# LRMPUT/PUTSLAM

Measured on AMD Instinct MI355X. Metric: frame-pairs/s (match+RANSAC+Kabsch), 640x480 @ 2000 kpts, higher is better.
Workload: dtype f32; 1 GPU; BASELINE configs[2]: TUM fr1/desk-style synthetic sequence, 500 frames = 499 frame pairs per step per GPU, 2000 kpts/frame, 256-bit descriptors, Hamming BF + cross-check -> depth filter -> H=4096 3-pt Umeyama hypotheses (fixed) scored with errorVersion 1 -> refit; inputs resident in HBM; kpts=2000, hypotheses=4096, world_size=1, force_dist=False, estimator=fixed, streams=4, join=end, submit=ps_batch_queue_submit: whole batches to the library's chains in turn, matcher_kernel=mfma-fused, score_kernel=fast, hw_queues=4, accepted_pairs=499

## Files before the change

putslam_amd/csrc/ps_capi.hip:

```cpp
#include "ps_kernels.h"
#include "ps_matcher_mfma.h"
#include "ps_score_fast.h"
#include "ps_score_euclid.h"
#include "ps_internal.h"
#include "ps_glue.h"

#include <cfloat>
#include <chrono>
#include <climits>
#include <cmath>
#include <cstdio>
#include <cstdlib>
#include <cstring>
#include <string>
#include <vector>

using namespace psdev;

static_assert(kPsReorderMargin == kReorderMargin && kPsReorderTopMax == kReorderTopMax, "ps_internal.h mirrors ps_score_fast.h");

namespace {

constexpr int kWidePairs = 16;
constexpr int kListRsplit3 = 4, kReorderGran = 64, kReorderC2div = 16;
// ... 81 lines not shown

int effective_mode(int errorVersion)
{
    switch (errorVersion) {
    case PS_EUCLIDEAN_ERROR:
    case PS_REPROJECTION_ERROR:
    case PS_EUCLIDEAN_AND_REPROJECTION_ERROR:
    case PS_ADAPTIVE_ERROR:
        return errorVersion;
    default:
        return PS_MAHALANOBIS_ERROR;
    }
}

enum class Scoring { Value, Euclid, Reproj };

struct Plan {
    int mode = 0;
    Scoring score = Scoring::Value;
    int H = 0;
    int minRun = 3;
    ScoreConsts sc{};
    FastConsts fc{};
    EuclidConsts ec{};
    PrepArgs pa{};
    SelectArgs sa{};
    ModelArgs ma{};
    int msplit = 1;
    bool genSplit = false;
    bool genPlain = false;
    bool reorder = false;
    bool prune = false;
    bool bailWatch = false;
    int bailSlot = 0;
    int prefix = 0;
    int lastStage = 0;
    bool big0 = false;
};

int make_plan(PsContext *ctx, const PsRansacParams *prm, const PsRansacConfig *cfg, const float *K, int cap,
              int trainRange, Plan &pl)
{
    if (!prm || !cfg) return fail(ctx, PS_ERR_BAD_ARG, "null params/config");
    if (prm->usedPairs != 3) return fail(ctx, PS_ERR_UNSUPPORTED, "usedPairs must be 3");
    if (cfg->numHypotheses < 1 || cfg->numHypotheses > PS_MAX_HYPOTHESES)
        return fail(ctx, PS_ERR_BAD_ARG, "numHypotheses out of range");
    if (cfg->estimator < PS_EST_RANSAC || cfg->estimator > PS_EST_FIXED)
        return fail(ctx, PS_ERR_BAD_ARG, "unknown estimator");
    pl.mode = effective_mode(prm->errorVersion);
    if (ctx->scoreFast == 0 || pl.mode == PS_MAHALANOBIS_ERROR) pl.score = Scoring::Value;
    else pl.score = (pl.mode == PS_EUCLIDEAN_ERROR || pl.mode == PS_ADAPTIVE_ERROR) ? Scoring::Euclid : Scoring::Reproj;
    float k[9] = {0, 0, 0, 0, 0, 0, 0, 0, 0};
    if (K) memcpy(k, K, sizeof k);
    pl.sc.fx = k[0]; pl.sc.fy = k[4]; pl.sc.cx = k[2]; pl.sc.cy = k[5];
    pl.sc.boundR = sq_bound_f64(prm->inlierThresholdReprojection);
    pl.sc.bLo = -1.0f;
    pl.sc.bHi = INFINITY;
    if (pl.sc.boundR >= 1e-20 && pl.sc.boundR <= 1e30) {
        const double w = 4.76837158203125e-07;
        double lo = pl.sc.boundR * (1.0 - w), hi = pl.sc.boundR * (1.0 + w);
        float flo = (float)lo, fhi = (float)hi;
        if ((double)flo > lo) flo = std::nextafterf(flo, 0.0f);
        if ((double)fhi < hi) fhi = std::nextafterf(fhi, INFINITY);
        pl.sc.bLo = flo;
        pl.sc.bHi = fhi;
    }
    {
        FastConsts &fc = pl.fc;
        const double fm = std::fmax(std::fmax(std::fabs((double)k[0]), std::fabs((double)k[4])), 1.0);
        const double cm = std::fmax(std::fabs((double)k[2]), std::fabs((double)k[5]));
        const double bR = pl.sc.boundR;
        fc.enabled = (bR >= 1e-12 && bR <= 1e12 && fm <= 1e6 && cm <= 1e6) ? 1 : 0;
        if (fc.enabled) {
            const double T = std::sqrt(bR);
            auto up = [](double v) { float f = (float)v; return (double)f < v ? std::nextafterf(f, INFINITY) : f; };
            auto down = [](double v) { float f = (float)v; return (double)f > v ? std::nextafterf(f, -INFINITY) : f; };
            fc.fmaxK = up(fm);
            fc.cmaxK = up(cm);
            fc.thrUp = up(T * (1.0 + 1e-5));
            fc.bIn0 = down(bR * (1.0 - 20.0 * 5.9604644775390625e-08));
            fc.cIn = up(2.0 * std::sqrt(2.0) * T * (1.0 + 1e-5));
            const double c = std::sqrt(2.0) * (1.0 + 1e-5);
            fc.thr2Up = up((double)fc.thrUp * (double)fc.thrUp);
            fc.cHi = up((2.0 * c + c * c) * (double)fc.thrUp);
        }
    }
    {
        EuclidConsts &ec = pl.ec;
        const double thr = prm->inlierThresholdEuclidean;
        ec.enabled = (thr >= 1e-10 && thr <= 1e10) ? 1 : 0;
        ec.tbLo = ec.tbHi = 0.0f;
        if (ec.enabled) {
            const double u = 5.9604644775390625e-08;
            auto up = [](double v) { float f = (float)v; return (double)f < v ? std::nextafterf(f, INFINITY) : f; };
            auto down = [](double v) { float f = (float)v; return (double)f > v ? std::nextafterf(f, -INFINITY) : f; };
            if (pl.mode == PS_ADAPTIVE_ERROR) {
                ec.tbLo = down(thr * (1.0 - 7.0 * u));
                ec.tbHi = up(thr * (1.0 + 7.0 * u));
            } else {
                const double Tb = std::sqrt((double)sq_bound_f32(thr));
                ec.tbLo = down(Tb * (1.0 - 6.0 * u));
                ec.tbHi = up(Tb * (1.0 + 6.0 * u));
            }
        }
    }
    pl.pa.fx = k[0]; pl.pa.fy = k[4]; pl.pa.cx = k[2]; pl.pa.cy = k[5];
    pl.pa.thrE = prm->inlierThresholdEuclidean;
    pl.pa.mode = pl.mode;
    pl.pa.cap = cap;
    pl.sa.estimator = cfg->estimator;
    pl.sa.mode = pl.mode;
    pl.sa.cap = cap;
    pl.sa.minMatches = (cfg->estimator == PS_EST_USAC) ? 8 : prm->minimalNumberOfMatches;
    pl.sa.minRatio = prm->minimalInlierRatioThreshold;
    pl.sa.trainRange = trainRange;
    pl.minRun = pl.sa.minMatches > 3 ? pl.sa.minMatches : 3;
    int H = cfg->numHypotheses;
    if (cfg->estimator == PS_EST_RANSAC) {
        int a = ransac_iterations_host(0.20), b = ransac_iterations_host(prm->minimalInlierRatioThreshold);
        int most = a > b ? a : b;
        if (most < H) H = most;
        if (H < 1) H = 1;
    } else if (cfg->estimator == PS_EST_USAC) {
        if (H > (int)kUsacMaxHyp) H = (int)kUsacMaxHyp;
    }
    pl.H = H;
    pl.sa.H = H;
    int rc = prepare_tables(ctx, cfg->estimator, prm->minimalInlierRatioThreshold, H, pl.sa);
    if (rc != PS_OK) return rc;
    if (pl.sa.iter0 > H) pl.sa.iter0 = H;
    pl.ma.seed = cfg->seed;
    pl.ma.raw = nullptr;
    pl.ma.seedDev = nullptr;
    return PS_OK;
}

void tick(PsContext *ctx, int slot, bool stop)
{
    if (!ctx->timing || slot >= kMaxTimed || ctx->ev.empty()) return;
    (void)hipEventRecord(ctx->ev[((size_t)ctx->curCall * kMaxTimed + slot) * 2 + (stop ? 1 : 0)], ctx->stream);
    if (stop) {
        ctx->slotMask[ctx->curCall] |= 1u << slot;
        if (slot + 1 > ctx->nTimed) ctx->nTimed = slot + 1;
    }
}

RecPtrs rec_ptrs(PsContext *ctx, Scoring score)
{
    RecPtrs r;
    r.G = score == Scoring::Euclid ? (float *)ctx->recF.p : nullptr;
    r.A = (float4 *)ctx->recA.p; r.B = (float4 *)ctx->recB.p; r.C = (float4 *)ctx->recC.p; r.D = (int4 *)ctx->recD.p;
    r.E = (float4 *)ctx->recE.p;
    r.F = (float2 *)ctx->recF.p;
#ifdef PS_STREAM_DIAG
    r.S = (float4 *)ctx->recShadow.p;
#endif
    return r;
}

int pick_split(long long blocksWithout, int maxSplit, int minChunkOf, int total)
{
    const long long want = 2048;
    if (blocksWithout >= want) return 1;
    long long s = (want + blocksWithout - 1) / (blocksWithout > 0 ? blocksWithout : 1);
    if (s > maxSplit) s = maxSplit;
    while (s > 1 && total / s < minChunkOf) --s;
    return (int)(s < 1 ? 1 : s);
}

template <int MODE>
void launch_score(PsContext *ctx, dim3 grid, const Plan &pl, int cap, int msplit)
{
    hipLaunchKernelGGL(ps_ransac_score<MODE>, grid, dim3(kBlock), 0, ctx->stream, (const float4 *)ctx->recA.p,
                       (const float4 *)ctx->recB.p, (const float4 *)ctx->recC.p, (const int32_t *)ctx->mvalid.p,
                       (const float2 *)ctx->cmax.p, pl.ma, pl.sc, pl.H, cap, pl.minRun, msplit, (int32_t *)ctx->counts.p);
}

unsigned big_limit(int mode) { return mode == PS_REPROJECTION_ERROR ? 1536u : 1280u; }

int prepare_score(PsContext *ctx, Plan &pl, int P, int cap, bool complete = false, bool adaptive = false, const void *dataKey = nullptr)
{
    const int H = pl.H;
    const int hb = (H + kBlock - 1) / kBlock;
    const bool prunable = pl.score != Scoring::Value;
    const size_t mbytes = (size_t)P * H * 12 * sizeof(float);
    pl.prefix = pl.sa.estimator == PS_EST_FIXED ? kPrefixFixed : kPrefixAdaptive;
    if (ctx->forcePrefix > 0 && pl.sa.estimator == PS_EST_FIXED) pl.prefix = ctx->forcePrefix;
    const double units = (double)P * (double)(hb - 1) * (double)cap;
    const StagedFrom sf = pl.score == Scoring::Euclid ? (pl.sa.estimator == PS_EST_FIXED ? kStagedFromEuclidFixed : kStagedFromEuclidAdaptive)
                                                      : (pl.sa.estimator == PS_EST_FIXED ? kStagedFromReprojFixed : kStagedFromReprojAdaptive);
    double stagedFrom = sf.base + sf.perRow * (double)cap;
    if (ctx->sideBySide >= 2) {
        const StagedFrom sb = pl.score == Scoring::Euclid ? (pl.sa.estimator == PS_EST_FIXED ? kStagedFromEuclidFixedSbs : kStagedFromEuclidAdaptiveSbs)
                                                          : (pl.sa.estimator == PS_EST_FIXED ? kStagedFromReprojFixedSbs : kStagedFromReprojAdaptiveSbs);
        const double sbs = sb.base + sb.perRow * (double)cap;
        stagedFrom = ctx->sideBySide >= 3 ? sbs : std::sqrt(sbs * stagedFrom);
    }
    pl.prune = !complete && ctx->prune != 0 && prunable && H > kPrefixFixed && (ctx->prune == 2 || units >= stagedFrom);
    pl.bailWatch = false;
    pl.bailSlot = 0;
    const bool willReorder = ctx->reorder == 1 || (ctx->reorder == 2 && pl.sa.estimator == PS_EST_FIXED);
    if (adaptive && pl.prune && willReorder && ctx->bail != 0 && pl.score == Scoring::Euclid && pl.sa.estimator == PS_EST_FIXED) {
        if (!ctx->bailHost) {
            const size_t nb = (size_t)PsContext::kBailKinds * 2 * sizeof(unsigned);
            if (hipHostMalloc((void **)&ctx->bailHost, nb, hipHostMallocMapped) == hipSuccess &&
                hipHostGetDevicePointer((void **)&ctx->bailHostDev, ctx->bailHost, 0) == hipSuccess) {
                memset(ctx->bailHost, 0, nb);
                if (ensure(ctx, ctx->bailCnt, nb) == PS_OK) (void)hipMemsetAsync(ctx->bailCnt.p, 0, nb, ctx->stream);
            } else {
                (void)hipGetLastError();
                ctx->bailHostDev = nullptr;
            }
        }
        if (ctx->bailHostDev && ctx->bailCnt.p) {
            int pclass = 0;
            for (int q = P; q > 1; q >>= 1) ++pclass;
            int slot = -1, lru = 0;
            for (int i = 0; i < PsContext::kBailKinds; ++i) {
                const PsContext::BailKind &b = ctx->bailKinds[i];
                if (b.mode == pl.mode && b.estimator == pl.sa.estimator && b.H == H && b.pclass == pclass && b.cap == cap && b.frames == dataKey) slot = i;
                if (b.used < ctx->bailKinds[lru].used) lru = i;
            }
            if (slot < 0) {
                slot = lru;
                PsContext::BailKind &b = ctx->bailKinds[slot];
                b.mode = pl.mode; b.estimator = pl.sa.estimator; b.H = H; b.pclass = pclass; b.cap = cap; b.frames = dataKey;
                b.hopeless = 0;
                b.calls = 0;
                (void)hipStreamSynchronize(ctx->stream);
                b.seen[0] = ((volatile unsigned *)ctx->bailHost)[2 * slot];
                b.seen[1] = ((volatile unsigned *)ctx->bailHost)[2 * slot + 1];
            }
            PsContext::BailKind &b = ctx->bailKinds[slot];
            b.used = ++ctx->bailClock;
            const unsigned s0 = ((volatile unsigned *)ctx->bailHost)[2 * slot], s1 = ((volatile unsigned *)ctx->bailHost)[2 * slot + 1];
            if (s0 != b.seen[0]) {
                const unsigned d0 = s0 - b.seen[0], d1 = s1 - b.seen[1];
                const int was = b.hopeless;
                b.hopeless = (2ull * d1 > d0) ? 1 : 0;
                if (b.hopeless != was) b.calls = 0;
                b.seen[0] = s0;
                b.seen[1] = s1;
            }
            if (b.hopeless && (++b.calls & 15) != 0)
                pl.prune = false;
            pl.bailWatch = pl.prune;
            pl.bailSlot = slot;
            ctx->bailSlot = slot;
            ctx->hopeless = b.hopeless;
        }
    }
    if (adaptive && !pl.prune && (double)P * (double)H * (double)cap > 2.0e14)
        return fail(ctx, PS_ERR_UNSUPPORTED, "complete scoring of this batch (pairs x hypotheses x matches > 2e14) would run for minutes: "
                                             "leave the staged scoring on (option \"prune\") or pass fewer pairs per call");
    PS_ENSURE(ctx->counts, (size_t)P * H * sizeof(int32_t));
    pl.msplit = pick_split((long long)P * (pl.prune ? 1 : hb), 32, 64, cap);
    pl.genSplit = pl.prune && ctx->genSplit != 0 && pl.msplit > 1;
    if (pl.genSplit) pl.msplit = pl.msplit * 2 < 32 ? pl.msplit * 2 : 32;
    if (ctx->forceMsplit > 0) pl.msplit = ctx->forceMsplit;
    if (pl.msplit <= 1) pl.genSplit = false;
    pl.pa.zeroCounts = pl.msplit > 1 ? (int32_t *)ctx->counts.p : nullptr;
    pl.pa.zeroH = pl.prune ? pl.prefix : H;
    pl.pa.zeroStride = H;
    pl.ma.models = nullptr;
    pl.ma.modelH = H;
    pl.lastStage = (pl.sa.estimator != PS_EST_FIXED && !willReorder && ctx->singleRest != 0) ? 1 : kStages;
    if (pl.prune) {
        const size_t room = ctx->modelRoomMiB > 0 ? ((size_t)ctx->modelRoomMiB << 20)
                                                  : (pl.sa.estimator == PS_EST_FIXED ? ((size_t)2 << 30) : ((size_t)256 << 20));
        if (mbytes > room) {
            long long fit = (long long)(room / ((size_t)P * 12 * sizeof(float))) & ~(long long)(kBlock - 1);
            pl.ma.modelH = (int)(fit < kPrefixFixed ? kPrefixFixed : fit);
        }
    }
    if ((P <= kWidePairs && mbytes <= ((size_t)64 << 20)) || pl.prune) {
        PS_ENSURE(ctx->models, (size_t)P * pl.ma.modelH * 12 * sizeof(float));
        pl.ma.models = (float *)ctx->models.p;
    }
    pl.genPlain = false;
    if (!pl.prune && pl.score != Scoring::Value && ctx->genSplit != 0 && pl.msplit > 1 && P >= kGenPlainFrom && mbytes <= ((size_t)1 << 30)) {
        PS_ENSURE(ctx->models, mbytes);
        pl.ma.models = (float *)ctx->models.p;
        PS_ENSURE(ctx->validMask, (size_t)P * ((H + 63) / 64) * sizeof(unsigned long long));
        pl.genPlain = true;
    }
    pl.pa.zeroSurvA = pl.pa.zeroSurvB = nullptr;
    pl.big0 = (unsigned)pl.msplit * (unsigned)P * (pl.prune ? 1u : (unsigned)hb) > big_limit(pl.mode);
    pl.pa.skipF = !(pl.score == Scoring::Reproj && (pl.prune || pl.big0));
    pl.pa.skipE = !(pl.score == Scoring::Reproj && !pl.big0);
    if (pl.prune) {
        if (pl.lastStage > 1) {
            PS_ENSURE(ctx->survA, (size_t)P * pl.ma.modelH * sizeof(int32_t));
            PS_ENSURE(ctx->survB, (size_t)P * pl.ma.modelH * sizeof(int32_t));
        }
        PS_ENSURE(ctx->survN, (size_t)2 * P * sizeof(int32_t));
        if (pl.genSplit) PS_ENSURE(ctx->validMask, (size_t)P * ((pl.prefix + 63) / 64) * sizeof(unsigned long long));
        pl.reorder = ctx->reorder == 1 || (ctx->reorder == 2 && pl.sa.estimator == PS_EST_FIXED);
        if (pl.reorder) {
            const size_t n = (size_t)P * cap;
            PS_ENSURE(ctx->recF2, n * 40 > (size_t)P * ((cap + 1) / 2) * 64 ? n * 40 : (size_t)P * ((cap + 1) / 2) * 64);
            PS_ENSURE(ctx->permBuf, n * sizeof(int32_t));
            PS_ENSURE(ctx->prefInfo, (size_t)4 * P * sizeof(int32_t));
            PS_ENSURE(ctx->frontRec, (size_t)P * ((cap + 1) / 2) * 10 * sizeof(float));
        }
        pl.pa.zeroSurvA = (int32_t *)ctx->survN.p;
        pl.pa.zeroSurvB = (int32_t *)ctx->survN.p + P;
    }
    ctx->lastModelH = pl.ma.models ? pl.ma.modelH : 0;
    ctx->stagedP = pl.prune ? P : 0;
    ctx->stagedCap = pl.prune ? cap : 0;
    ctx->reorderedP = (pl.prune && pl.reorder) ? P : 0;
    return PS_OK;
}

struct K3Call {
    PsContext *ctx;
    const Plan &pl;
    int P, cap;
    const float2 *hotF;
    unsigned long long *dbg;
};

template <int KIND, bool LOOP = false> struct Kind {};

template <int MODE> struct EuclidK3 {
    const K3Call &c;
    template <int KIND, bool LOOP> void operator()(Kind<KIND, LOOP>, const StageArgs &st, unsigned groups, int msplit) const
    {
        PsContext *ctx = c.ctx;
        hipLaunchKernelGGL((ps_ransac_score_euclid<MODE, KIND, LOOP>), dim3(groups * (unsigned)msplit * (unsigned)c.P), dim3(kBlock),
                           0, ctx->stream, (const float4 *)ctx->recA.p, (const float4 *)ctx->recB.p,
                           KIND >= 1 ? c.hotF : (const float2 *)ctx->recF.p, (const int32_t *)ctx->mvalid.p,
                           (const float2 *)ctx->cmax.p, c.pl.ma, c.pl.sc, c.pl.ec, c.pl.sa, st, c.pl.H, c.cap, c.pl.minRun, msplit,
                           (int32_t *)ctx->counts.p, c.dbg);
    }
};

template <int MODE> struct ReprojK3 {
    const K3Call &c;
    template <bool BIG, int KIND, bool LOOP> void launch(const StageArgs &st, unsigned groups, int msplit) const
    {
        PsContext *ctx = c.ctx;
        hipLaunchKernelGGL((ps_ransac_score_fast<MODE, BIG, KIND, LOOP>), dim3(groups * (unsigned)msplit * (unsigned)c.P),
                           dim3(kBlock), 0, ctx->stream, (const float4 *)ctx->recA.p, (const float4 *)ctx->recB.p,
                           (const float4 *)ctx->recC.p, st.frontRec ? (const float4 *)st.frontRec : (const float4 *)ctx->recE.p,
                           KIND >= 1 ? c.hotF : (const float2 *)ctx->recF.p, (const int32_t *)ctx->mvalid.p,
                           (const float2 *)ctx->cmax.p, c.pl.ma, c.pl.sc, c.pl.fc, c.pl.ec, c.pl.sa, st, c.pl.H, c.cap, c.pl.minRun,
                           msplit, (int32_t *)ctx->counts.p, c.dbg);
    }
    template <int KIND, bool LOOP> void operator()(Kind<KIND, LOOP>, const StageArgs &st, unsigned groups, int msplit) const
    {
        if constexpr (KIND == 0) {
            if (!c.pl.big0) return launch<false, KIND, LOOP>(st, groups, msplit);
        }
        launch<true, KIND, LOOP>(st, groups, msplit);
    }
};

template <int MODE, class K3> void score_schedule(const K3Call &c, const K3 &k3)
{
    PsContext *ctx = c.ctx;
    const Plan &pl = c.pl;
    const int P = c.P;
    auto groups = [](int hCount) { return (unsigned)((hCount + kBlock - 1) / kBlock); };
    if (!pl.prune) {
        StageArgs st{};
        st.hCount = pl.H;
        if (pl.genPlain) {
            st.validMask = (unsigned long long *)ctx->validMask.p;
            st.genOnly = 1;
            k3(Kind<0>{}, st, groups(pl.H), 1);
            st.genOnly = 0;
        }
        k3(Kind<0>{}, st, groups(pl.H), pl.msplit);
        return;
    }
    auto list_groups = [&](int stage) {
        const int listed = (pl.H < pl.ma.modelH ? pl.H : pl.ma.modelH) - pl.prefix;
        const int all = ((listed > 0 ? listed : 1) + kBlock - 1) / kBlock;
        const int auto3 = all / 8 > 1 ? all / 8 : 1;
        const int auto2 = pl.score == Scoring::Euclid ? (all / 8 > 2 ? all / 8 : 2) : 64;
        const int want = pl.reorder ? (stage == 2 ? (ctx->listGroups2 > 0 ? ctx->listGroups2 : auto2)
                                                  : auto3) : all;
        return want < all ? want : all;
    };
    auto list_rsplit = [&](int stage) { return (pl.reorder && stage == kStages) ? kListRsplit3 : 1; };
    const bool usePretest = pl.reorder && ctx->pretest != 0 &&
                            (pl.mode == PS_EUCLIDEAN_AND_REPROJECTION_ERROR || pl.mode == PS_REPROJECTION_ERROR);
    const int blocks1 = (pl.H - pl.prefix + kBlock - 1) / kBlock;
    int loopGroups = 0;
    if (pl.sa.estimator != PS_EST_FIXED && blocks1 > 64) {
        loopGroups = (4096 + P - 1) / P;
        loopGroups = loopGroups < 4 ? 4 : loopGroups;
        loopGroups = loopGroups > blocks1 ? blocks1 : loopGroups;
    }
    auto stage_args = [&](int stage) {
        StageArgs st{};
        st.stage = stage;
        st.hBase = stage == 0 ? 0 : pl.prefix;
        st.hCount = stage == 0 ? pl.prefix : pl.H - pl.prefix;
        if (stage >= 2) st.hCount = list_groups(stage) * kBlock;
        int32_t *nA = (int32_t *)ctx->survN.p, *nB = nA + P;
        if (stage == 1) { st.listOut = (int32_t *)ctx->survA.p; st.countOut = nA; }
        if (stage == 2) { st.listIn = (const int32_t *)ctx->survA.p; st.countIn = nA; st.listOut = (int32_t *)ctx->survB.p; st.countOut = nB; }
        if (stage == 3) { st.listIn = (const int32_t *)ctx->survB.p; st.countIn = nB; }
        if (stage >= 1 && pl.reorder) st.perm = (const int32_t *)ctx->permBuf.p;
        if (stage >= 1 && pl.reorder) st.prefInfo = (const int32_t *)ctx->prefInfo.p;
        if (stage == 1 && usePretest) st.frontRec = (const float2 *)ctx->frontRec.p;
        st.listStride = pl.ma.modelH;
        st.loopGroups = stage == 1 ? loopGroups : 0;
        st.single = pl.lastStage == 1 ? 1 : 0;
        st.margin = ctx->reorderMargin;
        st.gran = kReorderGran;
        st.c2div = kReorderC2div;
        return st;
    };
    auto stage0_args = [&](bool gen) {
        StageArgs st = stage_args(0);
        if (pl.genSplit) {
            st.validMask = (unsigned long long *)ctx->validMask.p;
            st.genOnly = gen ? 1 : 0;
        }
        return st;
    };
    if (pl.genSplit) k3(Kind<0>{}, stage0_args(true), groups(pl.prefix), 1);
    k3(Kind<0>{}, stage0_args(false), groups(pl.prefix), pl.msplit);
    if (pl.reorder)
        hipLaunchKernelGGL(ps_stage_reorder<MODE>, dim3((unsigned)P), dim3(kBlock), 0, ctx->stream, (const float4 *)ctx->recA.p,
                           (const float4 *)ctx->recB.p, (const float4 *)ctx->recC.p, (const float2 *)ctx->recF.p,
                           (const int32_t *)ctx->mvalid.p, pl.ma, pl.sc, pl.sa, pl.prefix, ctx->reorderTop,
                           (ctx->bail != 0 && pl.score == Scoring::Euclid) ? 64 : 0, ctx->reorderMargin, pl.H, c.cap, pl.minRun,
                           (const int32_t *)ctx->counts.p, (float2 *)ctx->recF2.p, (int32_t *)ctx->permBuf.p,
                           (int32_t *)ctx->prefInfo.p, usePretest ? (float2 *)ctx->frontRec.p : (float2 *)nullptr,
                           pl.bailWatch ? (unsigned *)ctx->bailCnt.p + 2 * pl.bailSlot : (unsigned *)nullptr);
    if (loopGroups > 0)
        k3(Kind<1, true>{}, stage_args(1), (unsigned)loopGroups, 1);
    else
        k3(Kind<1>{}, stage_args(1), groups(pl.H - pl.prefix), 1);
    for (int sg = 2; sg <= pl.lastStage; ++sg) k3(Kind<2>{}, stage_args(sg), (unsigned)list_groups(sg), list_rsplit(sg));
}

template <int MODE> void launch_k3(const K3Call &c)
{
    if constexpr (MODE == PS_EUCLIDEAN_ERROR || MODE == PS_ADAPTIVE_ERROR) {
        if (c.pl.score == Scoring::Euclid) return score_schedule<MODE>(c, EuclidK3<MODE>{c});
    }
    if constexpr (MODE == PS_REPROJECTION_ERROR || MODE == PS_EUCLIDEAN_AND_REPROJECTION_ERROR) {
        if (c.pl.score == Scoring::Reproj) return score_schedule<MODE>(c, ReprojK3<MODE>{c});
    }
    launch_score<MODE>(c.ctx, dim3((unsigned)((c.pl.H + kBlock - 1) / kBlock) * (unsigned)c.pl.msplit * (unsigned)c.P), c.pl, c.cap,
                       c.pl.msplit);
}

int run_ransac_stage(PsContext *ctx, const Plan &pl, int P, int cap, const PsDMatch *dMatches,
                     const int32_t *dNumMatches, int matchStride, float *dPose, uint8_t *dMask, PsRansacStats *dStats,
                     int slot0)
{
    PS_ENSURE(ctx->counts, (size_t)P * pl.H * sizeof(int32_t));
    PS_ENSURE(ctx->idxList, (size_t)P * cap * sizeof(int32_t));
    tick(ctx, slot0, false);
    unsigned long long *dbg = nullptr;
    if (ctx->scoreStats && pl.score != Scoring::Value) {
        PS_ENSURE(ctx->dbgCnt, 8 * sizeof(unsigned long long));
        PS_HIP(hipMemsetAsync(ctx->dbgCnt.p, 0, 8 * sizeof(unsigned long long), ctx->stream));
        dbg = (unsigned long long *)ctx->dbgCnt.p;
    }
    const K3Call c{ctx, pl, P, cap, (const float2 *)(pl.reorder ? ctx->recF2.p : ctx->recF.p), dbg};
    switch (pl.mode) {
    case PS_EUCLIDEAN_ERROR: launch_k3<PS_EUCLIDEAN_ERROR>(c); break;
    case PS_REPROJECTION_ERROR: launch_k3<PS_REPROJECTION_ERROR>(c); break;
    case PS_EUCLIDEAN_AND_REPROJECTION_ERROR: launch_k3<PS_EUCLIDEAN_AND_REPROJECTION_ERROR>(c); break;
    case PS_ADAPTIVE_ERROR: launch_k3<PS_ADAPTIVE_ERROR>(c); break;
    default: launch_k3<PS_MAHALANOBIS_ERROR>(c); break;
    }
    tick(ctx, slot0, true);
    PS_HIP(hipGetLastError());
    SelectArgs sa = pl.sa;
    const size_t bitmapBytes = (((2 * (size_t)((sa.trainRange + 31) / 32)) + 3) & ~(size_t)3) * sizeof(uint32_t);
    const size_t stageRoom = ((size_t)63 << 10) - bitmapBytes;
    sa.stageCap = cap < 1536 ? cap : 1536;
    if ((size_t)sa.stageCap * 32 > stageRoom) sa.stageCap = (int)(stageRoom / 32);
    size_t lds = bitmapBytes + (size_t)sa.stageCap * 8 * sizeof(float);
    tick(ctx, slot0 + 1, false);
    hipLaunchKernelGGL(ps_select_refit<kBlock>, dim3((unsigned)P), dim3(kBlock), lds, ctx->stream,
                       (const float4 *)ctx->recA.p, (const float4 *)ctx->recB.p, (const float4 *)ctx->recC.p,
                       (const int4 *)ctx->recD.p, (const int32_t *)ctx->mvalid.p, (const int32_t *)ctx->counts.p,
                       dMatches, dNumMatches, matchStride, pl.ma, pl.sc, sa, (int32_t *)ctx->idxList.p, dPose,
                       dMask, dStats, ctx->stampsOn ? (unsigned long long *)ctx->stamps.p : (unsigned long long *)nullptr,
                       (pl.bailWatch && pl.reorder) ? (const unsigned *)ctx->bailCnt.p + 2 * pl.bailSlot : (const unsigned *)nullptr,
                       (pl.bailWatch && pl.reorder) ? ctx->bailHostDev + 2 * pl.bailSlot : (unsigned *)nullptr);
    tick(ctx, slot0 + 1, true);
    PS_HIP(hipGetLastError());
    return PS_OK;
}

int ensure_records(PsContext *ctx, size_t P, size_t cap)
{
    const size_t n = P * cap;
    PS_ENSURE(ctx->recA, n * 16);
    PS_ENSURE(ctx->recB, n * 16);
    PS_ENSURE(ctx->recC, n * 16);
    PS_ENSURE(ctx->recD, n * 16);
    PS_ENSURE(ctx->recE, n * 16);
    PS_ENSURE(ctx->recF, n * 40 > P * ((cap + 1) / 2) * 64 ? n * 40 : P * ((cap + 1) / 2) * 64);
#ifdef PS_STREAM_DIAG
    static const bool shadow = std::getenv("PUTSLAM_HIP_DIAG_SHADOW_RECORDS") != nullptr && std::atoi(std::getenv("PUTSLAM_HIP_DIAG_SHADOW_RECORDS")) != 0;
    if (shadow) PS_ENSURE(ctx->recShadow, n * 7 * 16);
#endif
    return PS_OK;
}

template <bool REC, int BLK>
void launch_prep(PsContext *ctx, const PsFrameSet &fs, const int32_t *dPairs, int P, const PrepArgs &pa, const RecPtrs &rp,
                 PsDMatch *dMatches, int32_t *dNumMatches)
{
    hipLaunchKernelGGL((ps_crosscheck_prep<REC, BLK>), dim3((unsigned)P), dim3(BLK), (size_t)fs.maxKpts * sizeof(uint32_t), ctx->stream,
                       fs.pts, fs.nkpts, dPairs, (uint32_t *)ctx->keys.p, pa, dMatches, dNumMatches, rp, (int32_t *)ctx->mvalid.p,
                       (float2 *)ctx->cmax.p, ctx->stampsOn ? (unsigned long long *)ctx->stamps.p : (unsigned long long *)nullptr);
}

int run_match_stage(PsContext *ctx, const PsFrameSet &fs, const int32_t *dPairs, int P, const Plan *pl, PsDMatch *dMatches,
                    int32_t *dNumMatches, int slot0)
{
    const int cap = fs.maxKpts;
    FrameStrides strides;
    if (int rc = frame_strides(ctx, fs, true, fs.pts != nullptr, "frame set", strides)) return rc;
    const int fstrideDw = strides.descDwords();
    PrepArgs pa = pl ? pl->pa : PrepArgs{};
    if (!pl) pa.cap = cap;
    pa.ptsStride = strides.ptsFloats();
    PS_ENSURE(ctx->keys, (size_t)P * cap * sizeof(uint32_t));
    PS_ENSURE(ctx->mvalid, (size_t)P * sizeof(int32_t));
    PS_ENSURE(ctx->cmax, (size_t)P * sizeof(float2));
    if (pl) {
        int rc = ensure_records(ctx, (size_t)P, (size_t)cap);
        if (rc != PS_OK) return rc;
    }
    const bool useMfma = ctx->matcher == 1 || (ctx->matcher == 2 && (double)P * cap * cap > 2.0e7);
    ctx->matcherUsed = useMfma ? 1 : 0;
    const size_t keyBytes = (size_t)P * cap * sizeof(uint32_t);
    const size_t cleanBefore = ctx->keysCleanPtr == ctx->keys.p ? ctx->keysCleanBytes : 0;
    struct KeysInUse {
        PsContext *c;
        size_t restore;
        bool done = false;
        ~KeysInUse() { c->keysCleanBytes = done ? restore : 0; }
    } keysInUse{ctx, cleanBefore};
    if (useMfma) {
        constexpr int TT = kMfmaTT;
        const int tpf = (cap + kTileRows - 1) / kTileRows;
        const int groups = (tpf + kWavesPerWG * TT - 1) / (kWavesPerWG * TT);
        int qsplit = pick_split((long long)P * groups, tpf, 1, tpf);
        if (ctx->forceQsplit > 0) qsplit = ctx->forceQsplit < tpf ? ctx->forceQsplit : tpf;
        if (ctx->matcherFused) {
            if (ctx->forceQsplit <= 0 && (long long)P * groups >= 1024) qsplit = 1;
            if (qsplit > 1) {
                int rc = keys_clean(ctx, keyBytes);
                if (rc != PS_OK) return rc;
                keysInUse.restore = ctx->keysCleanBytes;
            }
            tick(ctx, 5, false);
            hipLaunchKernelGGL(ps_hamming_mfma_fused<TT>, dim3((unsigned)(groups * qsplit) * (unsigned)P), dim3(kBlock), 0,
                               ctx->stream, (const uint32_t *)fs.desc, fs.nkpts, dPairs, cap, fstrideDw, tpf, groups, qsplit,
                               (uint32_t *)ctx->keys.p);
            tick(ctx, 5, true);
            PS_HIP(hipGetLastError());
        } else {
        PS_ENSURE(ctx->xq, (size_t)P * tpf * kTileU4 * sizeof(uint4));
        int xchunks = tpf < 8 ? tpf : 8;
        if ((long long)P * xchunks < 1024) xchunks = tpf < 64 ? tpf : 64;
        tick(ctx, 4, false);
        hipLaunchKernelGGL(ps_expand_query_fp4, dim3((unsigned)xchunks * (unsigned)P), dim3(kBlock), 0, ctx->stream,
                           (const uint32_t *)fs.desc, fs.nkpts, dPairs, cap, fstrideDw, tpf, xchunks, (uint4 *)ctx->xq.p,
                           qsplit > 1 ? (uint32_t *)ctx->keys.p : (uint32_t *)nullptr);
        tick(ctx, 4, true);
        tick(ctx, 5, false);
        hipLaunchKernelGGL(ps_hamming_mfma<TT>, dim3((unsigned)(groups * qsplit) * (unsigned)P), dim3(kBlock), 0,
                           ctx->stream, (const uint32_t *)fs.desc, fs.nkpts, dPairs, cap, fstrideDw, tpf, groups, qsplit,
                           (const uint4 *)ctx->xq.p, (uint32_t *)ctx->keys.p);
        tick(ctx, 5, true);
        PS_HIP(hipGetLastError());
        }
    } else {
        constexpr int TPL = 2;
        const int tiles = (cap + kBlock * TPL - 1) / (kBlock * TPL);
        int qsplit = pick_split((long long)P * tiles, 128, 16, cap);
        if (ctx->forceQsplit > 0) qsplit = ctx->forceQsplit;
        if (qsplit > 1) {
            int rc = keys_clean(ctx, keyBytes);
            if (rc != PS_OK) return rc;
            keysInUse.restore = ctx->keysCleanBytes;
        }
        tick(ctx, slot0, false);
        hipLaunchKernelGGL(ps_hamming_nn<TPL>, dim3((unsigned)(tiles * qsplit) * (unsigned)P), dim3(kBlock), 0, ctx->stream,
                           (const uint4 *)fs.desc, fs.nkpts, dPairs, cap, strides.descUint4(), tiles, qsplit, (uint32_t *)ctx->keys.p);
        tick(ctx, slot0, true);
        PS_HIP(hipGetLastError());
    }
    tick(ctx, slot0 + 1, false);
    const bool wide = P <= kWidePairs;
    const auto prep = pl ? (wide ? launch_prep<true, 1024> : launch_prep<true, kBlock>)
                         : (wide ? launch_prep<false, 1024> : launch_prep<false, kBlock>);
    prep(ctx, fs, dPairs, P, pa, pl ? rec_ptrs(ctx, pl->score) : RecPtrs{}, dMatches, dNumMatches);
    tick(ctx, slot0 + 1, true);
    PS_HIP(hipGetLastError());
    keysInUse.done = true;
    return PS_OK;
}

void identity16(float *T)
{
    for (int i = 0; i < 16; ++i) T[i] = (i % 5 == 0) ? 1.0f : 0.0f;
}

}

extern "C" {

int ps_match_hamming256(PsContext *ctx, const uint8_t *query, int nq, size_t qstep, const uint8_t *train, int nt,
                        size_t tstep, PsDMatch *out, int *nout)
{
    int rc = bind(ctx);
    if (rc) return rc;
    TimingOff toff(ctx);
    if (nout) *nout = 0;
    if (!out || !nout || nq < 0 || nt < 0 || (nq > 0 && !query) || (nt > 0 && !train))
        return fail(ctx, PS_ERR_BAD_ARG, "ps_match_hamming256: bad argument");
    if ((nq > 0 && qstep < PS_DESC_BYTES) || (nt > 0 && tstep < PS_DESC_BYTES))
        return fail(ctx, PS_ERR_UNSUPPORTED, "descriptor rows must be 32 bytes (ORB/LDB); float descriptors are out of scope");
    if (nq > PS_MAX_KPTS || nt > PS_MAX_KPTS) return fail(ctx, PS_ERR_UNSUPPORTED, "more than PS_MAX_KPTS rows");
    if (nq == 0 || nt == 0) return PS_OK;
    int cap = nq > nt ? nq : nt;
    PS_ENSURE(ctx->sDesc, (size_t)2 * cap * 32);
    PS_ENSURE(ctx->sNk, 2 * sizeof(int32_t) + 2 * sizeof(int32_t));
    PS_ENSURE(ctx->sMatches, (size_t)cap * sizeof(PsDMatch));
    PS_ENSURE(ctx->sNumM, sizeof(int32_t));
    uint8_t *dDesc = (uint8_t *)ctx->sDesc.p;
    PS_HIP(hipMemcpy2DAsync(dDesc, 32, query, qstep, 32, (size_t)nq, hipMemcpyHostToDevice, ctx->stream));
    PS_HIP(hipMemcpy2DAsync(dDesc + (size_t)cap * 32, 32, train, tstep, 32, (size_t)nt, hipMemcpyHostToDevice,
                            ctx->stream));
    int32_t hostMeta[4] = {nq, nt, 0, 1};
    PS_HIP(hipMemcpyAsync(ctx->sNk.p, hostMeta, sizeof hostMeta, hipMemcpyHostToDevice, ctx->stream));
    PsFrameSet fs;
    fs.desc = dDesc;
    fs.pts = nullptr;
    fs.nkpts = (const int32_t *)ctx->sNk.p;
    fs.numFrames = 2;
    fs.maxKpts = cap;
    fs.descFrameStride = fs.ptsFrameStride = 0;
    rc = run_match_stage(ctx, fs, (const int32_t *)ctx->sNk.p + 2, 1, nullptr, (PsDMatch *)ctx->sMatches.p, (int32_t *)ctx->sNumM.p, 0);
    if (rc) return rc;
    int32_t n = 0;
    PS_HIP(hipMemcpyAsync(&n, ctx->sNumM.p, sizeof n, hipMemcpyDeviceToHost, ctx->stream));
    PS_HIP(hipStreamSynchronize(ctx->stream));
    if (n > 0) {
        PS_HIP(hipMemcpyAsync(out, ctx->sMatches.p, (size_t)n * sizeof(PsDMatch), hipMemcpyDeviceToHost, ctx->stream));
        PS_HIP(hipStreamSynchronize(ctx->stream));
    }
    *nout = n;
    return PS_OK;
}

static int ransac_host_entry(PsContext *ctx, const PsRansacParams *params, const PsRansacConfig *cfg, const float *K,
                             const float *prev, int nprev, const float *cur, int ncur, const PsDMatch *matches, int m,
                             float *pose, PsDMatch *inliers, int *ninl, uint8_t *mask, PsRansacStats *stats,
                             int32_t *countsOut)
{
    int rc = bind(ctx);
    if (rc) return rc;
    TimingOff toff(ctx);
    PsRansacStats st;
    memset(&st, 0, sizeof st);
    st.bestHypothesis = -1;
    st.numMatchesIn = m > 0 ? m : 0;
    st.pointInlierRatio = NAN;
    if (pose) identity16(pose);
    if (ninl) *ninl = 0;
    if (stats) *stats = st;
    if (!pose || !ninl || m < 0 || nprev < 0 || ncur < 0 || (m > 0 && (!matches || !prev || !cur || !inliers)))
        return fail(ctx, PS_ERR_BAD_ARG, "ps_ransac_rigid3d: bad argument");
    if (mask && m > 0) memset(mask, 0, (size_t)m);
    if (m > (1 << 22)) return fail(ctx, PS_ERR_UNSUPPORTED, "too many matches");
    for (int i = 0; i < m; ++i)
        if (matches[i].queryIdx < 0 || matches[i].queryIdx >= nprev || matches[i].trainIdx < 0 ||
            matches[i].trainIdx >= ncur)
            return fail(ctx, PS_ERR_BAD_ARG, "match index out of range");
    const int cap = m > 0 ? m : 1;
    const int trainRange = ncur <= 65536 ? ncur : 0;
    Plan pl;
    rc = make_plan(ctx, params, cfg, K, cap, trainRange, pl);
    if (rc) return rc;
    if (cfg->sampleIdx) {
        PS_ENSURE(ctx->raw, (size_t)pl.H * 3 * sizeof(uint32_t));
        PS_HIP(hipMemcpyAsync(ctx->raw.p, cfg->sampleIdx, (size_t)pl.H * 3 * sizeof(uint32_t), hipMemcpyHostToDevice,
                              ctx->stream));
        pl.ma.raw = (const uint32_t *)ctx->raw.p;
    }
    rc = prepare_score(ctx, pl, 1, cap, countsOut != nullptr);
    if (rc) return rc;
    PS_ENSURE(ctx->sMisc0, (size_t)(nprev > 0 ? nprev : 1) * 12);
    PS_ENSURE(ctx->sMisc1, (size_t)(ncur > 0 ? ncur : 1) * 12);
    PS_ENSURE(ctx->sMatches, (size_t)cap * sizeof(PsDMatch));
    PS_ENSURE(ctx->sNumM, sizeof(int32_t));
    PS_ENSURE(ctx->sMask, (size_t)cap);
    PS_ENSURE(ctx->sPose, 16 * sizeof(float));
    PS_ENSURE(ctx->sStats, sizeof(PsRansacStats));
    PS_ENSURE(ctx->mvalid, sizeof(int32_t));
    PS_ENSURE(ctx->cmax, sizeof(float2));
    rc = ensure_records(ctx, 1, (size_t)cap);
    if (rc) return rc;
    if (nprev > 0) PS_HIP(hipMemcpyAsync(ctx->sMisc0.p, prev, (size_t)nprev * 12, hipMemcpyHostToDevice, ctx->stream));
    if (ncur > 0) PS_HIP(hipMemcpyAsync(ctx->sMisc1.p, cur, (size_t)ncur * 12, hipMemcpyHostToDevice, ctx->stream));
    if (m > 0)
        PS_HIP(hipMemcpyAsync(ctx->sMatches.p, matches, (size_t)m * sizeof(PsDMatch), hipMemcpyHostToDevice,
                              ctx->stream));
    int32_t mm = m;
    PS_HIP(hipMemcpyAsync(ctx->sNumM.p, &mm, sizeof mm, hipMemcpyHostToDevice, ctx->stream));
    hipLaunchKernelGGL(ps_prep_from_matches, dim3(1), dim3(kBlock), 0, ctx->stream, (const float *)ctx->sMisc0.p,
                       (const float *)ctx->sMisc1.p, (const PsDMatch *)ctx->sMatches.p, m, pl.pa, rec_ptrs(ctx, pl.score),
                       (int32_t *)ctx->mvalid.p, (float2 *)ctx->cmax.p);
    PS_HIP(hipGetLastError());
    rc = run_ransac_stage(ctx, pl, 1, cap, (const PsDMatch *)ctx->sMatches.p, (const int32_t *)ctx->sNumM.p, cap,
                          (float *)ctx->sPose.p, (uint8_t *)ctx->sMask.p, (PsRansacStats *)ctx->sStats.p, 2);
    if (rc) return rc;
    std::vector<uint8_t> hmask((size_t)cap);
    PS_HIP(hipMemcpyAsync(pose, ctx->sPose.p, 16 * sizeof(float), hipMemcpyDeviceToHost, ctx->stream));
    PS_HIP(hipMemcpyAsync(&st, ctx->sStats.p, sizeof st, hipMemcpyDeviceToHost, ctx->stream));
    if (m > 0) PS_HIP(hipMemcpyAsync(hmask.data(), ctx->sMask.p, (size_t)m, hipMemcpyDeviceToHost, ctx->stream));
    if (countsOut) {
        int32_t mv = 0;
        PS_HIP(hipMemcpyAsync(&mv, ctx->mvalid.p, sizeof mv, hipMemcpyDeviceToHost, ctx->stream));
        PS_HIP(hipStreamSynchronize(ctx->stream));
        if (mv >= pl.minRun)
            PS_HIP(hipMemcpyAsync(countsOut, ctx->counts.p, (size_t)pl.H * sizeof(int32_t), hipMemcpyDeviceToHost,
                                  ctx->stream));
        else
// ... 296 lines not shown
```

putslam_amd/csrc/ps_context.cpp:

```cpp
#include <cfloat>
#include <climits>
#include <cmath>
#include <cstdio>
#include <cstdlib>
#include <cstring>

#include "ps_internal.h"

int ransac_iterations_host(double inlierRatio, double successProbability, int numberOfPairs)
{
    double v = std::log(1 - successProbability) / std::log(1 - std::pow(inlierRatio, numberOfPairs));
    if (!(v < 2147483647.0)) return INT_MAX;
    if (v < 0) return 0;
    return (int)v;
}

unsigned usac_stopping_host(double prob_good_model)
{
    if (prob_good_model < DBL_EPSILON) return kUsacMaxHyp;
    if (1 - prob_good_model < DBL_EPSILON) return 1;
    double n = std::log(1 - 0.99) / std::log(1 - prob_good_model);
    return (unsigned)std::ceil(n);
}

void build_ransac_table(double minRatio, int H, std::vector<float> &tab, int &iter0, float &tiny)
{
    uint32_t tlo = 0, thi;
    {
        float probe = 1e-4f;
        memcpy(&thi, &probe, 4);
        while (thi - tlo > 1) {
            uint32_t mid = tlo + (thi - tlo) / 2;
            float mf;
            memcpy(&mf, &mid, 4);
            if (ransac_iterations_host((double)mf) == 0) tlo = mid; else thi = mid;
        }
        memcpy(&tiny, &tlo, 4);
    }
    int itersMin = ransac_iterations_host(minRatio);
    int kcap = itersMin < H ? itersMin : H;
    if (kcap < 0) kcap = 0;
    tab.resize((size_t)kcap);
    uint32_t one;
    float onef = 1.0f;
    memcpy(&one, &onef, 4);
    uint32_t hi = one;
    for (int k = 0; k < kcap; ++k) {
        uint32_t lo = thi;
        while (hi - lo > 1) {
            uint32_t mid = lo + (hi - lo) / 2;
            float mf;
            memcpy(&mf, &mid, 4);
            if (ransac_iterations_host((double)mf) <= k) hi = mid; else lo = mid;
        }
        memcpy(&tab[(size_t)k], &hi, 4);
    }
    int i0 = ransac_iterations_host(0.20);
    iter0 = i0 < H ? i0 : H;
}

void build_usac_table(int H, std::vector<double> &tab)
{
    int n = H < (int)kUsacMaxHyp ? H : (int)kUsacMaxHyp;
    tab.resize((size_t)(n > 0 ? n : 0));
    uint64_t oneb;
    double oned = 1.0;
    memcpy(&oneb, &oned, 8);
    uint64_t hiPrev = oneb;
    const double pFloor = 1.862645149230957e-09;
    uint64_t floorb;
    memcpy(&floorb, &pFloor, 8);
    for (int k = 0; k < n; ++k) {
        unsigned target = (unsigned)k + 1u;
        uint64_t lo = floorb, hi = hiPrev;
        if (target >= kUsacMaxHyp) {
            tab[(size_t)k] = 0.0;
            continue;
        }
        {
            const double ps = -std::expm1(std::log(1 - 0.99) / (double)target);
            const double a = ps * (1.0 - 1e-11), b = ps * (1.0 + 1e-11);
            uint64_t ab, bb;
            memcpy(&ab, &a, 8);
            memcpy(&bb, &b, 8);
            if (ab > lo && ab < hi && usac_stopping_host(a) > target) lo = ab;
            if (bb > lo && bb < hi && usac_stopping_host(b) <= target) hi = bb;
        }
        while (hi - lo > 1) {
            uint64_t mid = lo + (hi - lo) / 2;
            double md;
            memcpy(&md, &mid, 8);
            if (usac_stopping_host(md) <= target) hi = mid; else lo = mid;
        }
        memcpy(&tab[(size_t)k], &hi, 8);
        hiPrev = hi;
    }
}


namespace {

struct OptDesc {
    const char *name;
    const char *env;
    int PsContext::*field;
    int lo, hi;
    const char *what;
    bool shape = false;
};
const OptDesc kOptions[] = {
    {"matcher", "MATCHER", &PsContext::matcher, 0, 2, "matcher: 0 (VALU), 1 (MFMA) or 2 (by batch size)"},
    {"matcher_fused", "MATCHER_FUSED", &PsContext::matcherFused, 0, 1, "matcher_fused: 0 or 1"},
    {"matcher_l2", "MATCHER_L2", &PsContext::matcherL2, 0, 1, "matcher_l2: 0 (value-exact sweep) or 1 (matrix-core prefilter + value-exact evaluation)"},
    {"l2_stats", nullptr, &PsContext::l2Stats, 0, 1, "l2_stats: 0 or 1"},
    {"score", "SCORE", &PsContext::scoreFast, 0, 1, "score: 0 (value-exact kernels) or 1 (decision-exact kernels)"},
    {"score_stats", nullptr, &PsContext::scoreStats, 0, 1, "score_stats: 0 or 1"},
    {"prune", "PRUNE", &PsContext::prune, 0, 2, "prune: 0 (complete scoring), 1 (staged from the cost model's batch size on) or 2 (staged whenever possible)"},
    {"side_by_side", "SIDE_BY_SIDE", &PsContext::sideBySide, 0, 16, "side_by_side: 0 (the context runs alone) or the number of launch chains it shares the chip with"},
    {"reorder", "REORDER", &PsContext::reorder, 0, 2, "reorder: 0, 1 or 2"},
    {"qsplit", "QSPLIT", &PsContext::forceQsplit, 0, 1024, "qsplit: 0 (automatic) .. 1024", true},
    {"msplit", "MSPLIT", &PsContext::forceMsplit, 0, 1024, "msplit: 0 (automatic) .. 1024", true},
    {"gensplit", "GENSPLIT", &PsContext::genSplit, 0, 1, "gensplit: 0 (stage 0 as one launch) or 1 (models, then the sweep)", true},
    {"singlerest", "SINGLEREST", &PsContext::singleRest, 0, 1, "singlerest: 0 (three stages) or 1 (one stage after the prefix, adaptive schedules)", true},
    {"pretest", "PRETEST", &PsContext::pretest, 0, 1, "pretest: 0 or 1 (stage 1's one-direction pre-test)", true},
    {"list_g2", "LISTG2", &PsContext::listGroups2, 0, 64, "list_g2: 0 (automatic) .. 64 work-groups per pair of stage 2", true},
    {"prefix", "PREFIX", &PsContext::forcePrefix, 0, 256, "prefix: 0 (default) or 64, 128, 192, 256 hypotheses of stage 0 (fixed schedule)", true},
    {"reorder_top", "REORDER_TOP", &PsContext::reorderTop, 1, kPsReorderTopMax, "reorder_top: 1 .. 16 voters", true},
    {"reorder_margin", "REORDER_MARGIN", &PsContext::reorderMargin, 1, 4096, "reorder_margin: 1 .. 4096 matches", true},
    {"bail", "BAIL", &PsContext::bail, 0, 1, "bail: 0 or 1 (pairs whose prefix leaves nothing to abandon are swept in one stage)"},
    {"stream_copy_kernels", "STREAM_COPY_KERNELS", &PsContext::streamCopyKernels, 0, 1, "stream_copy_kernels: 0 (hipMemcpyAsync) or 1 (copy kernels over mapped pinned memory)"},
    {"stream_ahead", "STREAM_AHEAD", &PsContext::streamAhead, -1, 8, "stream_ahead: -1 (automatic: six places in all) or 0 .. 8 chunks the pipelined stream takes beyond one per lane (queued on the lanes' streams)"},
    {"model_room_mib", "MODEL_ROOM_MIB", &PsContext::modelRoomMiB, 0, 65536, "model_room_mib: 0 (default) .. 65536 MiB for the staged scoring's parked models"},
};
const OptDesc *find_option(const char *name)
{
    const bool dbg = strncmp(name, "debug.", 6) == 0;
    if (dbg) name += 6;
    for (const OptDesc &o : kOptions)
        if (o.shape == dbg && strcmp(name, o.name) == 0) return &o;
    return nullptr;
}
bool option_value_ok(const OptDesc &o, int v)
{
    if (v < o.lo || v > o.hi) return false;
    if (strcmp(o.name, "prefix") == 0) return (v & 63) == 0;
    return true;
}
int parse_option_text(const OptDesc &o, const char *v)
{
    if (strcmp(o.name, "score") == 0) {
        if (strcmp(v, "exact") == 0) return 0;
        if (strcmp(v, "fast") == 0) return 1;
    }
    if (strcmp(o.name, "matcher") == 0) {
        if (strcmp(v, "valu") == 0) return 0;
        if (strcmp(v, "mfma") == 0) return 1;
        if (strcmp(v, "auto") == 0) return 2;
    }
    char *end = nullptr;
    const long x = std::strtol(v, &end, 10);
    if (end == v || *end != '\0' || x < INT_MIN || x > INT_MAX) return INT_MIN;
    return (int)x;
}


}

int psi_options_snapshot(const PsContext *ctx, int *out, int cap)
{
    int n = 0;
    for (const OptDesc &o : kOptions)
        if (n < cap) out[n++] = ctx->*(o.field);
    return n;
}

extern "C" {

int ps_abi_version(void) { return PS_ABI_VERSION; }

size_t ps_abi_sizeof_dmatch(void) { return sizeof(PsDMatch); }
size_t ps_abi_sizeof_params(void) { return sizeof(PsRansacParams); }
size_t ps_abi_sizeof_config(void) { return sizeof(PsRansacConfig); }
size_t ps_abi_sizeof_stats(void) { return sizeof(PsRansacStats); }
size_t ps_abi_sizeof_frameset(void) { return sizeof(PsFrameSet); }
size_t ps_abi_sizeof_results(void) { return sizeof(PsPairResults); }
size_t ps_abi_sizeof_host_results(void) { return sizeof(PsHostPairResults); }

int ps_context_create(int device, PsContext **out)
{
    if (!out) return PS_ERR_BAD_ARG;
    *out = nullptr;
    int n = 0;
    hipError_t e = hipGetDeviceCount(&n);
    if (e != hipSuccess || n <= 0) return PS_ERR_NO_DEVICE;
    if (device < 0 || device >= n) return PS_ERR_BAD_ARG;
    if (hipSetDevice(device) != hipSuccess) return PS_ERR_HIP;
    PsContext *ctx = new PsContext();
    ctx->device = device;
    hipDeviceProp_t prop;
    if (hipGetDeviceProperties(&prop, device) == hipSuccess) {
        strncpy(ctx->arch, prop.gcnArchName, sizeof(ctx->arch) - 1);
    }
    if (hipStreamCreateWithFlags(&ctx->own, hipStreamNonBlocking) != hipSuccess) {
        delete ctx;
        return PS_ERR_HIP;
    }
    ctx->stream = ctx->own;
    for (const OptDesc &o : kOptions) {
        if (!o.env) continue;
        const std::string name = std::string("PUTSLAM_HIP_") + o.env;
        if (const char *v = std::getenv(name.c_str())) {
            const int x = parse_option_text(o, v);
            if (option_value_ok(o, x)) ctx->*(o.field) = x;
        }
    }
    psi_kernel_attributes();
    *out = ctx;
    return PS_OK;
}

void ps_context_destroy(PsContext *ctx)
{
    if (!ctx) return;
    (void)hipSetDevice(ctx->device);
    (void)hipStreamSynchronize(ctx->stream);
    Buf *all[] = {&ctx->keys, &ctx->recA, &ctx->recB, &ctx->recC, &ctx->recD, &ctx->recE, &ctx->recF, &ctx->recShadow, &ctx->models, &ctx->survA, &ctx->survB, &ctx->survN, &ctx->recF2, &ctx->permBuf, &ctx->prefInfo, &ctx->frontRec, &ctx->validMask, &ctx->stamps, &ctx->dbgCnt, &ctx->bailCnt, &ctx->counts, &ctx->mvalid,
                  &ctx->cmax, &ctx->idxList, &ctx->raw, &ctx->xq, &ctx->tabR, &ctx->tabU, &ctx->sDesc, &ctx->sNk,
                  &ctx->sMatches, &ctx->sNumM, &ctx->sMask, &ctx->sPose, &ctx->sStats,
                  &ctx->sMisc0, &ctx->sMisc1, &ctx->sMisc2, &ctx->exFlag, &ctx->exPar, &ctx->viewChunks, &ctx->levelTab, &ctx->poseSets, &ctx->loopPairs, &ctx->l2Keys, &ctx->l2Img, &ctx->l2Norms, &ctx->l2List, &ctx->l2ListLo, &ctx->l2Count, &ctx->l2Stat};
    for (Buf *b : all) release(*b);
    for (hipEvent_t e : ctx->ev)
        if (e) (void)hipEventDestroy(e);
    if (ctx->bailHost) (void)hipHostFree(ctx->bailHost);
    if (ctx->handoff) (void)hipEventDestroy(ctx->handoff);
    if (ctx->own) (void)hipStreamDestroy(ctx->own);
    delete ctx;
}

int ps_context_set_stream(PsContext *ctx, void *s)
{
    if (!ctx) return PS_ERR_BAD_ARG;
    hipStream_t next = s ? (hipStream_t)s : ctx->own;
    if (next == ctx->stream) return PS_OK;
    int rc = bind(ctx);
    if (rc) return rc;
    if (ctx->handoff && ctx->handoffPending) PS_HIP(hipStreamWaitEvent(next, ctx->handoff, 0));
    ctx->stream = next;
    return PS_OK;
}

void *ps_context_stream(PsContext *ctx) { return ctx ? (void *)ctx->stream : nullptr; }
int ps_context_device(const PsContext *ctx) { return ctx ? ctx->device : (int)PS_ERR_BAD_ARG; }

int ps_context_set_option(PsContext *ctx, const char *name, int value)
{
    if (!ctx || !name) return PS_ERR_BAD_ARG;
    if (strcmp(name, "stamps") == 0) {
        if (value != 0 && value != 1) return fail(ctx, PS_ERR_BAD_ARG, "stamps: 0 or 1");
        if (value) {
            int rc = bind(ctx);
            if (rc) return rc;
            PS_ENSURE(ctx->stamps, 16 * sizeof(unsigned long long));
            PS_HIP(hipMemsetAsync(ctx->stamps.p, 0, 16 * sizeof(unsigned long long), ctx->stream));
        }
        ctx->stampsOn = value;
        return PS_OK;
    }
    const OptDesc *o = find_option(name);
    if (!o) return fail(ctx, PS_ERR_BAD_ARG, "unknown option");
    if (!option_value_ok(*o, value)) return fail(ctx, PS_ERR_BAD_ARG, o->what);
    ctx->*(o->field) = value;
    if (strcmp(name, "bail") == 0) {
        for (PsContext::BailKind &b : ctx->bailKinds) b = PsContext::BailKind();
        ctx->hopeless = 0;
        ctx->bailSlot = -1;
    }
    return PS_OK;
}

int ps_context_get_option(const PsContext *ctx, const char *name)
{
    if (!ctx || !name) return PS_ERR_BAD_ARG;
    if (strcmp(name, "matcher_used") == 0) return ctx->matcherUsed;
    if (strcmp(name, "matcher_l2_used") == 0) return ctx->matcherL2Used;
    if (strcmp(name, "stamps") == 0) return ctx->stampsOn;
    if (strcmp(name, "last_staged_pairs") == 0) return ctx->stagedP;
    if (strcmp(name, "hopeless") == 0) return ctx->hopeless;
    if (strcmp(name, "arena_mib") == 0) {
        const Buf *all[] = {&ctx->keys, &ctx->recA, &ctx->recB, &ctx->recC, &ctx->recD, &ctx->recE, &ctx->recF, &ctx->models,
                            &ctx->survA, &ctx->survB, &ctx->survN, &ctx->recF2, &ctx->permBuf, &ctx->prefInfo, &ctx->frontRec,
                            &ctx->validMask, &ctx->stamps, &ctx->dbgCnt, &ctx->bailCnt, &ctx->counts, &ctx->mvalid, &ctx->cmax,
                            &ctx->idxList, &ctx->raw, &ctx->xq, &ctx->tabR, &ctx->tabU, &ctx->sDesc, &ctx->sNk, &ctx->sMatches,
                            &ctx->sNumM, &ctx->sMask, &ctx->sPose, &ctx->sStats, &ctx->sMisc0, &ctx->sMisc1, &ctx->sMisc2, &ctx->exFlag, &ctx->exPar, &ctx->viewChunks, &ctx->levelTab, &ctx->poseSets, &ctx->loopPairs, &ctx->l2Keys, &ctx->l2Img, &ctx->l2Norms, &ctx->l2List, &ctx->l2ListLo, &ctx->l2Count, &ctx->l2Stat};
        size_t sum = 0;
        for (const Buf *b : all) sum += b->cap;
        return (int)((sum + (((size_t)1 << 20) - 1)) >> 20);
    }
    if (strcmp(name, "hw_queues_seen") == 0) return psi_hw_queues_seen();
    if (strcmp(name, "last_model_slots") == 0) return ctx->lastModelH;
    if (strcmp(name, "last_reordered_pairs") == 0) return ctx->reorderedP;
    const OptDesc *o = find_option(name);
    return o ? ctx->*(o->field) : (int)PS_ERR_BAD_ARG;
}

int ps_context_synchronize(PsContext *ctx)
{
    int rc = bind(ctx);
    if (rc) return rc;
    PS_HIP(hipStreamSynchronize(ctx->stream));
    return PS_OK;
}

const char *ps_last_error(const PsContext *ctx) { return ctx ? ctx->err.c_str() : "null context"; }

void psi_set_error(PsContext *ctx, const char *what)
{
    if (ctx) ctx->err = what ? what : "";
}

void psi_copy_options(PsContext *dst, const PsContext *src)
{
    if (!dst || !src) return;
    for (const OptDesc &o : kOptions) dst->*(o.field) = src->*(o.field);
}
const char *ps_device_arch(const PsContext *ctx) { return ctx ? ctx->arch : ""; }

int ps_context_enable_timing(PsContext *ctx, int enable)
{
    int rc = bind(ctx);
    if (rc) return rc;
    if (enable && ctx->ev.empty()) {
        ctx->ev.assign((size_t)kTimingRing * kMaxTimed * 2, nullptr);
        for (hipEvent_t &e : ctx->ev) PS_HIP(hipEventCreate(&e));
    }
    ctx->timing = enable != 0;
    ctx->timedCalls = 0;
    ctx->curCall = 0;
    ctx->nTimed = 0;
    memset(ctx->slotMask, 0, sizeof ctx->slotMask);
    return PS_OK;
}

int ps_last_kernel_times_ms(PsContext *ctx, float *ms)
{
    int rc = bind(ctx);
    if (rc) return rc;
    if (!ctx->timing || ctx->timedCalls == 0) return 0;
    PS_HIP(hipStreamSynchronize(ctx->stream));
    for (int i = 0; i < ctx->nTimed; ++i) {
        float t = 0.f;
        size_t b = ((size_t)ctx->curCall * kMaxTimed + i) * 2;
        if (ctx->slotMask[ctx->curCall] & (1u << i)) PS_HIP(hipEventElapsedTime(&t, ctx->ev[b], ctx->ev[b + 1]));
        ms[i] = t;
    }
    return ctx->nTimed;
}

int ps_kernel_time_totals(PsContext *ctx, double *sum_ms, int *launches)
{
    int rc = bind(ctx);
    if (rc) return rc;
    for (int i = 0; i < kMaxTimed; ++i) {
        sum_ms[i] = 0.0;
        launches[i] = 0;
    }
    if (!ctx->timing || ctx->timedCalls == 0) return 0;
    PS_HIP(hipStreamSynchronize(ctx->stream));
    long long n = ctx->timedCalls < kTimingRing ? ctx->timedCalls : kTimingRing;
    for (long long c = 0; c < n; ++c)
        for (int i = 0; i < ctx->nTimed; ++i) {
            if (!(ctx->slotMask[c] & (1u << i))) continue;
            float t = 0.f;
            size_t b = ((size_t)c * kMaxTimed + i) * 2;
            PS_HIP(hipEventElapsedTime(&t, ctx->ev[b], ctx->ev[b + 1]));
            sum_ms[i] += t;
            launches[i] += 1;
        }
    return ctx->nTimed;
}

const char *ps_kernel_names(void)
{
    return "ps_hamming_nn\0ps_crosscheck_prep\0ps_ransac_score\0ps_select_refit\0ps_expand_query_fp4\0ps_hamming_mfma\0";
}

uint64_t ps_algorithmic_bytes(int nkpts, int matchesIn, int matchesValid, int H)
{
    return 2ull * nkpts * 32 + 16ull * matchesIn + 2ull * nkpts * 12 + 8ull * matchesValid + 12ull * H + 4ull * H +
           (uint64_t)matchesValid + 64ull;
}


int ps_predicted_level(int octave, double detDist, double curDist)
{
    const double scaleFactor = 1.2;
    const int nLevels = 8;
    const double logScaleFactor = std::log(scaleFactor);
    double detLevelScaleFactor = std::pow(scaleFactor, octave);
    double curLevelScaleFactor = detLevelScaleFactor * detDist / curDist;
    int curLevel = (int)std::ceil(std::log(curLevelScaleFactor) / logScaleFactor);
    if (curLevel < 0) curLevel = 0;
    if (curLevel > nLevels - 1) curLevel = nLevels - 1;
    return curLevel;
}

static bool level_above(double x, int k) { return std::ceil(std::log(x) / std::log(1.2)) > (double)k; }

int psi_level_tables(double *t7, double *pow64)
{
    static double T[7], P[PS_LEVEL_OCTAVE_MAX - PS_LEVEL_OCTAVE_MIN + 1];
    static int state = 0;
    if (state == 0) {
        auto bits = [](double d) { uint64_t b; std::memcpy(&b, &d, 8); return b; };
        auto val = [](uint64_t b) { double d; std::memcpy(&d, &b, 8); return d; };
        bool clean = true;
        for (int k = 0; k < 7 && clean; ++k) {
            uint64_t lo = bits(0.5), hi = bits(8.0);
            while (lo < hi) {
                const uint64_t mid = lo + (hi - lo) / 2;
                if (level_above(val(mid), k))
                    hi = mid;
                else
                    lo = mid + 1;
            }
            T[k] = val(lo);
            for (int64_t d = -4096; d <= 4096 && clean; ++d) clean = level_above(val(lo + (uint64_t)d), k) == (d >= 0);
        }
        for (int o = PS_LEVEL_OCTAVE_MIN; o <= PS_LEVEL_OCTAVE_MAX; ++o) P[o - PS_LEVEL_OCTAVE_MIN] = std::pow(1.2, o);
        state = clean ? 1 : -1;
    }
    if (state < 0) return PS_ERR_UNSUPPORTED;
    if (t7) std::memcpy(t7, T, sizeof(T));
    if (pow64) std::memcpy(pow64, P, sizeof(P));
    return PS_OK;
}

int ps_level_thresholds(double t[7])
{
    if (!t) return PS_ERR_BAD_ARG;
    return psi_level_tables(t, nullptr);
}

int ps_view_angles(const double *curPose16, const double *poses16, int numPoses, double *angle)
{
    if (!curPose16 || numPoses < 0 || (numPoses > 0 && (!poses16 || !angle))) return PS_ERR_BAD_ARG;
    const float a0 = (float)curPose16[8], a1 = (float)curPose16[9], a2 = (float)curPose16[10];
    const float na = std::sqrt(a0 * a0 + (a1 * a1 + a2 * a2));
    for (int q = 0; q < numPoses; ++q) {
        const double *m = poses16 + (size_t)q * 16;
        const float b0 = (float)m[8], b1 = (float)m[9], b2 = (float)m[10];
        const float dot = b0 * a0 + (b1 * a1 + b2 * a2);
        const float nb = std::sqrt(b0 * b0 + (b1 * b1 + b2 * b2));
        const float r = dot / (nb * na);
        angle[q] = std::fabs(std::acos((double)r));
    }
    return PS_OK;
}


}
```

putslam_amd/csrc/ps_internal.h:

```cpp
#pragma once
#include <hip/hip_runtime_api.h>

#include <cstddef>
#include <cstdint>
#include <string>
#include <vector>

#include "putslam_hip.h"

struct Buf {
    void *p = nullptr;
    size_t cap = 0;
};


constexpr int kMaxTimed = 8;
constexpr int kTimingRing = 128;

constexpr int kPsReorderMargin = 16, kPsReorderTopMax = 16;
constexpr unsigned kUsacMaxHyp = 850000u;

struct PsContext {
    int device = 0;
    hipStream_t own = nullptr;
    hipStream_t stream = nullptr;
    hipEvent_t handoff = nullptr;
    bool handoffPending = false;
    std::string err;
    char arch[64] = {0};
    Buf keys, recA, recB, recC, recD, recE, recF, counts, mvalid, cmax, idxList, raw;
    Buf models;
    Buf survA, survB, survN;
    Buf validMask;
    Buf frontRec;
    Buf prefInfo;
    Buf recF2, permBuf;
    Buf dbgCnt;
    Buf xq;
    Buf recShadow;
    Buf tabR, tabU;
    Buf sDesc, sNk, sMatches, sNumM, sMask, sPose, sStats, sMisc0, sMisc1, sMisc2;
    Buf exFlag, exPar;
    Buf viewChunks;
    Buf levelTab;
    Buf poseSets;
    Buf loopPairs;
    Buf l2Keys;
    Buf l2Img, l2Norms, l2List, l2ListLo, l2Count, l2Stat;
    int tabEstimator = -1, tabH = -1, tabRN = 0, tabUN = 0, tabIter0 = 0;
    double tabMinRatio = -1.0;
    float tabTiny = 0.0f;
    bool timing = false;
    std::vector<hipEvent_t> ev;
    long long timedCalls = 0;
    int curCall = 0;
    int nTimed = 0;
    unsigned slotMask[kTimingRing] = {0};
    int forceQsplit = 0, forceMsplit = 0;
    int matcher = 2;
    int matcherUsed = 1;
    int matcherFused = 1;
    int matcherL2 = 1;
    int matcherL2Used = 0;
    int l2Stats = 0;
    int scoreFast = 1;
    int scoreStats = 0;
    int prune = 1;
    int sideBySide = 0;
    int reorder = 2;
    int genSplit = 1;
    int singleRest = 1;
    int pretest = 1;
    int listGroups2 = 0;
    int forcePrefix = 0;
    int bail = 1;
    int streamCopyKernels = 1;
    int streamAhead = -1;
    int modelRoomMiB = 0;
    int reorderTop = 8, reorderMargin = kPsReorderMargin;
    int stampsOn = 0;
    Buf stamps;
    unsigned long long arenaGen = 0;
    int stagedP = 0, stagedCap = 0, reorderedP = 0;
    int lastModelH = 0;
    struct BailKind {
        int mode = -1, estimator = 0, H = 0, pclass = 0, cap = 0;
        const void *frames = nullptr;
        unsigned seen[2] = {0, 0};
        int hopeless = 0, calls = 0;
        unsigned long long used = 0;
    };
    static constexpr int kBailKinds = 8;
    BailKind bailKinds[kBailKinds];
    unsigned long long bailClock = 0;
    int bailSlot = -1;
    Buf bailCnt;
    unsigned *bailHost = nullptr;
    unsigned *bailHostDev = nullptr;
    int hopeless = 0;
    void *keysCleanPtr = nullptr;
    size_t keysCleanBytes = 0;
};


inline int fail(PsContext *c, int code, const char *what, hipError_t e = hipSuccess)
{
    if (c) {
        c->err = what;
        if (e != hipSuccess) {
            c->err += ": ";
            c->err += hipGetErrorString(e);
        }
    }
    return code;
}

#define PS_HIP(call)                                                  \
    do {                                                              \
        hipError_t e_ = (call);                                       \
        if (e_ != hipSuccess) return fail(ctx, PS_ERR_HIP, #call, e_); \
    } while (0)

inline int ensure(PsContext *ctx, Buf &b, size_t bytes)
{
    if (bytes <= b.cap) return PS_OK;
    size_t want = bytes + (bytes / 4 < ((size_t)16 << 20) ? bytes / 4 : ((size_t)16 << 20)) + 256;
    if (b.p) {
        hipError_t e = hipStreamSynchronize(ctx->stream);
        if (e != hipSuccess) return fail(ctx, PS_ERR_HIP, "hipStreamSynchronize", e);
        (void)hipFree(b.p);
        b.p = nullptr;
        b.cap = 0;
    }
    hipError_t e = hipMalloc(&b.p, want);
    if (e != hipSuccess) return fail(ctx, PS_ERR_ALLOC, "hipMalloc", e);
    b.cap = want;
    ctx->arenaGen++;
    return PS_OK;
}
#define PS_ENSURE(buf, bytes)                        \
    do {                                             \
        int rc_ = ensure(ctx, (buf), (bytes));       \
        if (rc_ != PS_OK) return rc_;                \
    } while (0)


inline void release(Buf &b)
{
    if (b.p) (void)hipFree(b.p);
    b.p = nullptr;
    b.cap = 0;
}


inline int bind(PsContext *ctx)
{
    if (!ctx) return PS_ERR_BAD_ARG;
    hipError_t e = hipSetDevice(ctx->device);
    if (e != hipSuccess) return fail(ctx, PS_ERR_HIP, "hipSetDevice", e);
    ctx->err.clear();
    return PS_OK;
}

int ransac_iterations_host(double inlierRatio, double successProbability = 0.98, int numberOfPairs = 3);
unsigned usac_stopping_host(double prob_good_model);
void build_ransac_table(double minRatio, int H, std::vector<float> &tab, int &iter0, float &tiny);
void build_usac_table(int H, std::vector<double> &tab);
int psi_options_snapshot(const PsContext *ctx, int *out, int cap);

extern "C" {
void psi_set_error(PsContext *ctx, const char *what);
void psi_copy_options(PsContext *dst, const PsContext *src);
int psi_hw_queues_seen(void);
int psi_hw_queues_defaulted(void);
void psi_kernel_attributes(void);
int psi_level_tables(double *t7, double *powTable);
}
```

putslam_amd/csrc/ps_kernels.h:

```cpp
#pragma once

#include "ps_device_math.h"

#include "../../include/putslam_hip.h"

namespace psdev {

constexpr int kBlock = 256;
constexpr uint32_t kNoKey = 0xFFFFFFFFu;

PS_D unsigned xcd_remap(unsigned L, unsigned total)
{
    const unsigned xcd = L & 7u, idx = L >> 3;
    const unsigned q = total >> 3, r = total & 7u;
    return (xcd < r ? xcd * (q + 1u) : r * (q + 1u) + (xcd - r) * q) + idx;
}

PS_D void phase_stamp(unsigned long long *stamps, int i)
{
    if (stamps != nullptr && threadIdx.x == 0 && blockIdx.x == 0) stamps[i] = __builtin_readcyclecounter();
}

PS_D uint32_t bcnt_acc(uint32_t x, uint32_t acc)
{
// ... 151 lines not shown
        const int sv = wsum[i];
        if (i < w) off += sv;
        tot += sv;
    }
    posA = (off & 0xFFFF) + __popcll(ba & below);
    posB = (off >> 16) + __popcll(bb & below);
    totalA = tot & 0xFFFF;
    totalB = tot >> 16;
}

template <int BLOCK = kBlock> PS_D void block_max2(float &a, float &b, float2 *red)
{
#pragma unroll
    for (int o = 32; o > 0; o >>= 1) {
        a = fmaxf(a, __shfl_down(a, o, 64));
        b = fmaxf(b, __shfl_down(b, o, 64));
    }
    if ((threadIdx.x & 63) == 0) red[threadIdx.x >> 6] = make_float2(a, b);
    __syncthreads();
    float2 r = red[0];
#pragma unroll
    for (int i = 1; i < BLOCK / 64; ++i) {
        r.x = fmaxf(r.x, red[i].x);
        r.y = fmaxf(r.y, red[i].y);
    }
    __syncthreads();
    a = r.x;
    b = r.y;
}

template <int BLOCK = kBlock> PS_D float block_max(float v, float *red)
{
#pragma unroll
    for (int o = 32; o > 0; o >>= 1) v = fmaxf(v, __shfl_down(v, o, 64));
    if ((threadIdx.x & 63) == 0) red[threadIdx.x >> 6] = v;
    __syncthreads();
    float r = red[0];
#pragma unroll
    for (int i = 1; i < BLOCK / 64; ++i) r = fmaxf(r, red[i]);
    __syncthreads();
    return r;
}

struct PrepArgs {
    float fx, fy, cx, cy;
    double thrE;
    int mode;
    int cap;
    int ptsStride;
    int32_t *zeroCounts;
    int zeroH;
    int zeroStride;
    int32_t *zeroSurvA, *zeroSurvB;
    int skipE, skipF;
};

struct RecPtrs {
    float4 *A;
    float4 *B;
    float4 *C;
    int4 *D;
    float4 *E;
#ifdef PS_STREAM_DIAG
    float4 *S;
#endif
    float2 *F;
    float *G;
};

PS_D float write_records(const PrepArgs &a, const RecPtrs &r, int p, int v, int srcIdx, int q, int t, float px, float py,
                         float pz, float cx_, float cy_, float cz_, float fixedBound)
{
    const float bound = a.mode == PS_ADAPTIVE_ERROR ? sq_bound_f32(a.thrE * (double)pz) : fixedBound;
    const size_t slot = (size_t)p * a.cap + (size_t)v;
    r.A[slot] = make_float4(px, py, pz, bound);
    r.B[slot] = make_float4(cx_, cy_, cz_, 1.0f);
    r.D[slot] = make_int4(srcIdx, q, t, 0);
    const bool euclidOnly = a.mode == PS_EUCLIDEAN_ERROR || a.mode == PS_ADAPTIVE_ERROR;
    float ou = 0.0f, ov = 0.0f, nu = 0.0f, nv = 0.0f;
    if (!euclidOnly) {
        project(px, py, pz, a.fx, a.fy, a.cx, a.cy, ou, ov);
        project(cx_, cy_, cz_, a.fx, a.fy, a.cx, a.cy, nu, nv);
        r.C[slot] = make_float4(ou, ov, nu, nv);
    }
    if (r.G != nullptr) {
        const bool adaptive = a.mode == PS_ADAPTIVE_ERROR;
        const int rf = adaptive ? 16 : 12;
        float *g = r.G + ((size_t)p * (size_t)((a.cap + 1) >> 1) + (size_t)(v >> 1)) * rf + (v & 1);
        if (adaptive) {
            const float w = 1.0f / pz;
            g[0] = cx_ * w; g[2] = cy_ * w; g[4] = cz_ * w; g[6] = w;
            g[8] = px * w; g[10] = py * w; g[12] = pz * w; g[14] = 0.0f;
        } else {
            g[0] = cx_; g[2] = cy_; g[4] = cz_;
            g[6] = px; g[8] = py; g[10] = pz;
        }
        return 0.0f;
    }
    if (euclidOnly) return 0.0f;
    const float4 e = make_float4(a.cx - ou, a.cx - nu, a.cy - ov, a.cy - nv);
    if (!a.skipE) r.E[slot] = e;
    if (!a.skipF) {
        float2 *f = r.F + 5 * slot;
        f[0] = make_float2(cx_, px); f[1] = make_float2(cy_, py); f[2] = make_float2(cz_, pz);
        f[3] = make_float2(e.x, e.y); f[4] = make_float2(e.z, e.w);
    }
#ifdef PS_STREAM_DIAG
    if (r.S != nullptr) {
        float4 *sh = r.S + 7 * slot;
        sh[0] = make_float4(px, py, pz, bound); sh[1] = make_float4(cx_, cy_, cz_, 1.0f); sh[2] = make_float4(ou, ov, nu, nv);
        sh[3] = make_float4((float)srcIdx, (float)q, (float)t, 0.0f); sh[4] = make_float4(cx_, px, cy_, py);
        sh[5] = make_float4(cz_, pz, e.x, e.y); sh[6] = make_float4(e.z, e.w, 0.0f, 0.0f);
    }
#endif
    const bool num = e.x == e.x && e.y == e.y && e.z == e.z && e.w == e.w;
    return num ? fmaxf(fmaxf(fabsf(e.x), fabsf(e.y)), fmaxf(fabsf(e.z), fabsf(e.w))) : INFINITY;
}

PS_D void finish_pair_records(const PrepArgs &a, const RecPtrs &r, int p, int M)
{
    if (r.G == nullptr || !(M & 1)) return;
    const int rf = a.mode == PS_ADAPTIVE_ERROR ? 16 : 12;
    float *g = r.G + ((size_t)p * (size_t)((a.cap + 1) >> 1) + (size_t)(M >> 1)) * rf;
    for (int i = 0; i < rf; i += 2) g[i + 1] = g[i];
}

template <bool WITH_RECORDS, int BLOCK = kBlock>
__global__ __launch_bounds__(BLOCK) void ps_crosscheck_prep(const float *__restrict__ pts,
                                                             const int32_t *__restrict__ nkpts,
                                                             const int32_t *__restrict__ pairs,
                                                             uint32_t *__restrict__ keys, PrepArgs a,
                                                             PsDMatch *__restrict__ matches,
                                                             int32_t *__restrict__ numMatches, RecPtrs rec,
                                                             int32_t *__restrict__ mvalid, float2 *__restrict__ cmaxOut,
                                                             unsigned long long *__restrict__ stamps)
{
    extern __shared__ __align__(16) uint32_t s_best[];
    phase_stamp(stamps, 0);
    __shared__ int s_wsum[2 * (BLOCK / 64)];
    __shared__ float2 s_red[BLOCK / 64];
    float cm = 0.0f;
    float um = 0.0f;
    const int p = blockIdx.x;
    const int cap = a.cap;
    const int fq = pairs[2 * p], ft = pairs[2 * p + 1];
    const int nq = nkpts[fq], nt = nkpts[ft];
    uint32_t k0 = kNoKey, k1 = kNoKey;
    if ((int)threadIdx.x < nt) k0 = keys[(size_t)p * cap + threadIdx.x];
    if ((int)threadIdx.x + BLOCK < nt) k1 = keys[(size_t)p * cap + threadIdx.x + BLOCK];
    for (int q = threadIdx.x; q < nq; q += BLOCK) s_best[q] = kNoKey;
    __syncthreads();
    for (int t = threadIdx.x; t < nt; t += BLOCK) {
        uint32_t key = t < BLOCK ? k0 : (t < 2 * BLOCK ? k1 : keys[(size_t)p * cap + t]);
        if (key != kNoKey) {
            uint32_t q = key & 0xFFFFu, d = key >> 16;
            atomicMin(&s_best[q], (d << 16) | (uint32_t)t);
            keys[(size_t)p * cap + t] = kNoKey;
        }
    }
    __syncthreads();
    phase_stamp(stamps, 1);
    const float *pp = pts + (size_t)fq * a.ptsStride;
    const float *cp = pts + (size_t)ft * a.ptsStride;
    int base = 0, vbase = 0;
    struct Cand {
        uint32_t key;
        float px, py, pz, cx, cy, cz;
    };
    auto fetch = [&](int q, Cand &c) {
        c.key = (q < nq) ? s_best[q] : kNoKey;
        c.px = c.py = c.pz = c.cx = c.cy = c.cz = 0.0f;
        if (WITH_RECORDS && c.key != kNoKey) {
            const int t = (int)(c.key & 0xFFFFu);
            c.px = pp[3 * q]; c.py = pp[3 * q + 1]; c.pz = pp[3 * q + 2];
            c.cx = cp[3 * t]; c.cy = cp[3 * t + 1]; c.cz = cp[3 * t + 2];
        }
    };
    const float fixedBound = (WITH_RECORDS && a.mode != PS_ADAPTIVE_ERROR) ? sq_bound_f32(a.thrE) : 0.0f;
    Cand cur;
    fetch((int)threadIdx.x, cur);
    int trip = 0;
    for (int q0 = 0; q0 < nq; q0 += BLOCK, ++trip) {
        const int q = q0 + threadIdx.x;
        Cand nxt;
        nxt.key = kNoKey;
        nxt.px = nxt.py = nxt.pz = nxt.cx = nxt.cy = nxt.cz = 0.0f;
        if (q0 + BLOCK < nq) fetch(q + BLOCK, nxt);
        const uint32_t key = cur.key;
        const bool has = key != kNoKey;
        const int t = (int)(key & 0xFFFFu);
        const float px = cur.px, py = cur.py, pz = cur.pz, cx_ = cur.cx, cy_ = cur.cy, cz_ = cur.cz;
        const bool ok = WITH_RECORDS && has && depth_ok(px, py, pz) && depth_ok(cx_, cy_, cz_);
        int pos, total, vpos, vtotal;
        block_scan_flags2_alt<BLOCK>(has, ok, pos, total, vpos, vtotal, s_wsum, trip);
        if (has) {
            PsDMatch m;
            m.queryIdx = q;
            m.trainIdx = t;
            m.imgIdx = 0;
            m.distance = (float)(key >> 16);
            matches[(size_t)p * cap + base + pos] = m;
        }
        if (WITH_RECORDS) {
            if (ok) {
                um = fmaxf(um, write_records(a, rec, p, vbase + vpos, base + pos, q, t, px, py, pz, cx_, cy_, cz_, fixedBound));
                cm = fmaxf(cm, fmaxf(fmaxf(fabsf(px), fabsf(py)), fmaxf(fabsf(pz), fmaxf(fabsf(cx_), fmaxf(fabsf(cy_), fabsf(cz_))))));
            }
            vbase += vtotal;
        }
        base += total;
        cur = nxt;
    }
    phase_stamp(stamps, 2);
    if (WITH_RECORDS) {
        float c = cm, u = um;
        block_max2<BLOCK>(c, u, s_red);
        if (threadIdx.x == 0) cmaxOut[p] = make_float2(c, u);
        if (threadIdx.x == 0) finish_pair_records(a, rec, p, vbase);
        if (a.zeroCounts)
            for (int i = threadIdx.x; i < a.zeroH; i += BLOCK) a.zeroCounts[(size_t)p * a.zeroStride + i] = 0;
    }
    if (threadIdx.x == 0) {
        numMatches[p] = base;
        if (WITH_RECORDS) mvalid[p] = vbase;
        if (WITH_RECORDS && a.zeroSurvA) {
            a.zeroSurvA[p] = 0;
            a.zeroSurvB[p] = 0;
        }
    }
    phase_stamp(stamps, 3);
}

__global__ __launch_bounds__(kBlock) void ps_prep_from_matches(const float *__restrict__ prev,
                                                               const float *__restrict__ cur,
                                                               const PsDMatch *__restrict__ matches, int m, PrepArgs a,
                                                               RecPtrs rec, int32_t *__restrict__ mvalid,
                                                               float2 *__restrict__ cmaxOut)
{
    __shared__ int s_wsum[kBlock / 64];
    __shared__ float s_red[kBlock / 64];
    float cm = 0.0f, um = 0.0f;
    int vbase = 0;
    const float fixedBound = a.mode != PS_ADAPTIVE_ERROR ? sq_bound_f32(a.thrE) : 0.0f;
    for (int i0 = 0; i0 < m; i0 += kBlock) {
        const int i = i0 + threadIdx.x;
        float px = 0, py = 0, pz = 0, cx_ = 0, cy_ = 0, cz_ = 0;
        int q = 0, t = 0;
        bool ok = false;
        if (i < m) {
            q = matches[i].queryIdx;
            t = matches[i].trainIdx;
            px = prev[3 * q]; py = prev[3 * q + 1]; pz = prev[3 * q + 2];
            cx_ = cur[3 * t]; cy_ = cur[3 * t + 1]; cz_ = cur[3 * t + 2];
            ok = depth_ok(px, py, pz) && depth_ok(cx_, cy_, cz_);
        }
        int vtotal;
        int vpos = block_scan_flag(ok, vtotal, s_wsum);
        if (ok) {
            um = fmaxf(um, write_records(a, rec, 0, vbase + vpos, i, q, t, px, py, pz, cx_, cy_, cz_, fixedBound));
            cm = fmaxf(cm, fmaxf(fmaxf(fabsf(px), fabsf(py)), fmaxf(fabsf(pz), fmaxf(fabsf(cx_), fmaxf(fabsf(cy_), fabsf(cz_))))));
        }
        vbase += vtotal;
    }
    float c = block_max(cm, s_red);
    float u = block_max(um, s_red);
    if (threadIdx.x == 0) {
        mvalid[0] = vbase;
        cmaxOut[0] = make_float2(c, u);
        finish_pair_records(a, rec, 0, vbase);
    }
    if (a.zeroCounts)
        for (int i = threadIdx.x; i < a.zeroH; i += kBlock) a.zeroCounts[i] = 0;
    if (threadIdx.x == 0 && a.zeroSurvA) {
        a.zeroSurvA[0] = 0;
        a.zeroSurvB[0] = 0;
    }
}

struct ModelArgs {
    uint64_t seed;
    const uint32_t *raw;
    const uint64_t *seedDev;
    float *models;
    int modelH;
};

PS_D void store_model(const ModelArgs &ma, size_t slot, const Rigid &m)
{
    float4 *d = reinterpret_cast<float4 *>(ma.models + slot * 12);
    d[0] = make_float4(m.R[0][0], m.R[0][1], m.R[0][2], m.R[1][0]);
    d[1] = make_float4(m.R[1][1], m.R[1][2], m.R[2][0], m.R[2][1]);
    d[2] = make_float4(m.R[2][2], m.t[0], m.t[1], m.t[2]);
}
PS_D void load_model(const ModelArgs &ma, size_t slot, Rigid &m)
{
    const float4 *d = reinterpret_cast<const float4 *>(ma.models + slot * 12);
    const float4 a = d[0], b = d[1], c = d[2];
    m.R[0][0] = a.x; m.R[0][1] = a.y; m.R[0][2] = a.z; m.R[1][0] = a.w;
    m.R[1][1] = b.x; m.R[1][2] = b.y; m.R[2][0] = b.z; m.R[2][1] = b.w;
    m.R[2][2] = c.x; m.t[0] = c.y; m.t[1] = c.z; m.t[2] = c.w;
}
PS_D uint64_t base_seed(const ModelArgs &ma) { return ma.seedDev ? *ma.seedDev : ma.seed; }

PS_D bool gen_model(const float4 *__restrict__ recA, const float4 *__restrict__ recB, size_t rbase, uint32_t M,
                    const ModelArgs &ma, uint64_t pairSeed, uint32_t h, Rigid &mdl)
{
    uint32_t idx[3];
    sample_triplet(pairSeed, ma.raw, h, M, idx);
    float src[3][3], dst[3][3];
#pragma unroll
    for (int j = 0; j < 3; ++j) {
        float4 A = recA[rbase + idx[j]];
        float4 B = recB[rbase + idx[j]];
        dst[j][0] = A.x; dst[j][1] = A.y; dst[j][2] = A.z;
        src[j][0] = B.x; src[j][1] = B.y; src[j][2] = B.z;
    }
    return umeyama3(src, dst, mdl);
}

struct ScoreConsts {
    float fx, fy, cx, cy;
    double boundR;
    float bLo, bHi;
};

constexpr float kDivLo = 9.094947017729282e-13f;
constexpr float kDivHi = 1.099511627776e12f;

PS_D void div2_shared(float a0, float a1, float b, float &q0, float &q1)
{
    float r0 = __builtin_amdgcn_rcpf(b);
    float e0 = __builtin_fmaf(-b, r0, 1.0f);
    float r1 = __builtin_fmaf(e0, r0, r0);
    float m0 = a0 * r1;
    float m1 = a1 * r1;
    float f0 = __builtin_fmaf(-b, m0, a0);
    float f1 = __builtin_fmaf(-b, m1, a1);
    float g0 = __builtin_fmaf(f0, r1, m0);
    float g1 = __builtin_fmaf(f1, r1, m1);
    float h0 = __builtin_fmaf(-b, g0, a0);
    float h1 = __builtin_fmaf(-b, g1, a1);
    q0 = __builtin_fmaf(h0, r1, g0);
    q1 = __builtin_fmaf(h1, r1, g1);
}

PS_D bool wave_all(bool p) { return __builtin_amdgcn_ballot_w64(p) == __builtin_amdgcn_ballot_w64(true); }

PS_D float min3_abs(float a, float b, float c)
{
    float r;
    asm("v_min3_f32 %0, |%1|, |%2|, |%3|" : "=v"(r) : "v"(a), "v"(b), "v"(c));
    return r;
}
PS_D float max3_abs(float a, float b, float c)
{
    float r;
    asm("v_max3_f32 %0, |%1|, |%2|, |%3|" : "=v"(r) : "v"(a), "v"(b), "v"(c));
    return r;
}
template <bool HI_HOISTED>
PS_D bool wave_div_window_ok(float a0, float a1, float b, float c0, float c1, float d)
{
    unsigned long long m = __builtin_amdgcn_ballot_w64(min3_abs(a0, a1, b) >= kDivLo) &
                           __builtin_amdgcn_ballot_w64(min3_abs(c0, c1, d) >= kDivLo);
    if (!HI_HOISTED)
        m &= __builtin_amdgcn_ballot_w64(max3_abs(a0, a1, b) <= kDivHi) &
             __builtin_amdgcn_ballot_w64(max3_abs(c0, c1, d) <= kDivHi);
    return m == __builtin_amdgcn_ballot_w64(true);
}

PS_D bool hi_bound_holds(const Rigid &m, float cmax, float fmaxK)
{
    float r = 0.0f, t = 0.0f;
#pragma unroll
    for (int i = 0; i < 3; ++i) {
#pragma unroll
        for (int j = 0; j < 3; ++j) r = fmaxf(r, fabsf(m.R[i][j]));
        t = fmaxf(t, fabsf(m.t[i]));
    }
    bool finite = true;
#pragma unroll
    for (int i = 0; i < 3; ++i) {
#pragma unroll
        for (int j = 0; j < 3; ++j) finite = finite && (m.R[i][j] == m.R[i][j]);
        finite = finite && (m.t[i] == m.t[i]);
    }
    const float e = (3.0f * r * cmax + t) * 1.01f;
    return finite && (e * fmaxK <= kDivHi);
}
PS_D int lanes_below(unsigned long long mask)
{
    return (int)__builtin_amdgcn_mbcnt_hi((uint32_t)(mask >> 32), __builtin_amdgcn_mbcnt_lo((uint32_t)mask, 0u));
}
PS_D unsigned long long uniform64(unsigned long long v)
{
    const uint32_t lo = (uint32_t)__builtin_amdgcn_readfirstlane((int)(uint32_t)v);
    const uint32_t hi = (uint32_t)__builtin_amdgcn_readfirstlane((int)(uint32_t)(v >> 32));
    return ((unsigned long long)hi << 32) | lo;
}
PS_D bool lane_in(unsigned long long mask)
{
    int x;
    asm("v_cndmask_b32 %0, 0, 1, %1" : "=v"(x) : "s"(mask));
    return x != 0;
}
PS_D void add_mask(int &cnt, unsigned long long mask)
{
    asm volatile("v_addc_co_u32 %0, vcc, 0, %0, %1" : "+v"(cnt) : "s"(mask) : "vcc");
}

PS_D bool div_window_ok(float a0, float a1, float b, float c0, float c1, float d)
{
    return min3_abs(a0, a1, b) >= kDivLo && min3_abs(c0, c1, d) >= kDivLo && max3_abs(a0, a1, b) <= kDivHi &&
           max3_abs(c0, c1, d) <= kDivHi;
}

template <int MODE>
PS_D bool inlier_test(const Rigid &mdl, const Rigid &inv, const ScoreConsts &k, const float4 &A, const float4 &B,
                      const float4 &C)
{
    float ex, ey, ez;
    xform(mdl, B.x, B.y, B.z, ex, ey, ez);
    bool in = true;
    if (MODE == PS_EUCLIDEAN_ERROR || MODE == PS_ADAPTIVE_ERROR || MODE == PS_EUCLIDEAN_AND_REPROJECTION_ERROR) {
        float d0 = ex - A.x, d1 = ey - A.y, d2 = ez - A.z;
        float s = d0 * d0 + (d1 * d1 + d2 * d2);
        in = s < A.w;
    }
    if (MODE == PS_REPROJECTION_ERROR || MODE == PS_EUCLIDEAN_AND_REPROJECTION_ERROR) {
        float nx, ny, nz;
        xform(inv, A.x, A.y, A.z, nx, ny, nz);
        float pnu, pnv, pou, pov;
        project(nx, ny, nz, k.fx, k.fy, k.cx, k.cy, pnu, pnv);
        project(ex, ey, ez, k.fx, k.fy, k.cx, k.cy, pou, pov);
        float dxn = pnu - C.z, dyn = pnv - C.w;
        float dxo = pou - C.x, dyo = pov - C.y;
        double e0 = (double)dxn * (double)dxn + (double)dyn * (double)dyn;
        double e1 = (double)dxo * (double)dxo + (double)dyo * (double)dyo;
        in = in && (e0 < k.boundR) && (e1 < k.boundR);
    }
    return in;
}

template <int MODE, bool HI_HOISTED>
PS_D void score_accumulate(const Rigid &mdl, const Rigid &inv, const ScoreConsts &k, const float4 &A, const float4 &B,
                           const float4 &C, int &cnt)
{
    float ex, ey, ez;
    xform(mdl, B.x, B.y, B.z, ex, ey, ez);
    bool in = true;
    if (MODE == PS_EUCLIDEAN_ERROR || MODE == PS_ADAPTIVE_ERROR || MODE == PS_EUCLIDEAN_AND_REPROJECTION_ERROR) {
        float d0 = ex - A.x, d1 = ey - A.y, d2 = ez - A.z;
        float s = d0 * d0 + (d1 * d1 + d2 * d2);
        in = s < A.w;
    }
    if (MODE == PS_REPROJECTION_ERROR || MODE == PS_EUCLIDEAN_AND_REPROJECTION_ERROR) {
        float nx, ny, nz;
        xform(inv, A.x, A.y, A.z, nx, ny, nz);
        float pnu, pnv, pou, pov;
        const float a0 = nx * k.fx, a1 = ny * k.fy, c0 = ex * k.fx, c1 = ey * k.fy;
        if (wave_div_window_ok<HI_HOISTED>(a0, a1, nz, c0, c1, ez)) {
            float q0, q1, q2, q3;
            div2_shared(a0, a1, nz, q0, q1);
            div2_shared(c0, c1, ez, q2, q3);
            pnu = q0 + k.cx; pnv = q1 + k.cy;
            pou = q2 + k.cx; pov = q3 + k.cy;
        } else {
            pnu = a0 / nz + k.cx; pnv = a1 / nz + k.cy;
            pou = c0 / ez + k.cx; pov = c1 / ez + k.cy;
        }
        float dxn = pnu - C.z, dyn = pnv - C.w;
        float dxo = pou - C.x, dyo = pov - C.y;
        float f0 = __builtin_fmaf(dxn, dxn, dyn * dyn), f1 = __builtin_fmaf(dxo, dxo, dyo * dyo);
        uint32_t u0, u1;
        memcpy(&u0, &f0, 4);
        memcpy(&u1, &f1, 4);
        uint32_t um = u0 > u1 ? u0 : u1;
        float fm;
        memcpy(&fm, &um, 4);
        const unsigned long long mIn = __builtin_amdgcn_ballot_w64(fm < k.bLo);
        const unsigned long long mOut = __builtin_amdgcn_ballot_w64(fm > k.bHi);
        if ((mIn | mOut) == __builtin_amdgcn_ballot_w64(true)) {
            if (MODE == PS_EUCLIDEAN_AND_REPROJECTION_ERROR)
                add_mask(cnt, mIn & __builtin_amdgcn_ballot_w64(in));
            else
                add_mask(cnt, mIn);
            return;
        }
        asm volatile("" : "+v"(dxn), "+v"(dyn), "+v"(dxo), "+v"(dyo));
        double e0 = (double)dxn * (double)dxn + (double)dyn * (double)dyn;
        double e1 = (double)dxo * (double)dxo + (double)dyo * (double)dyo;
        in = in && (e0 < k.boundR) && (e1 < k.boundR);
    }
    cnt += in ? 1 : 0;
}

template <int MODE>
__global__ __launch_bounds__(kBlock, 6) void ps_ransac_score(const float4 *__restrict__ recA,
                                                          const float4 *__restrict__ recB,
                                                          const float4 *__restrict__ recC,
                                                          const int32_t *__restrict__ mvalid,
                                                          const float2 *__restrict__ cmaxArr, ModelArgs ma,
                                                          ScoreConsts k, int H, int cap, int minRun, int msplit,
                                                          int32_t *__restrict__ counts)
{
    const unsigned hb = (unsigned)((H + kBlock - 1) / kBlock);
    const unsigned L = xcd_remap(blockIdx.x, gridDim.x);
    const unsigned bx = L % hb, by = (L / hb) % (unsigned)msplit;
    const int p = (int)(L / (hb * (unsigned)msplit));
    const int M = mvalid[p];
    if (M < minRun) return;
    const int h = (int)bx * kBlock + threadIdx.x;
    const size_t rbase = (size_t)p * cap;
    const int m0 = (int)(((long long)M * by) / msplit);
    const int m1 = (int)(((long long)M * (by + 1)) / msplit);

    Rigid mdl, inv;
    bool valid = false;
    if (h < H) {
        valid = gen_model(recA, recB, rbase, (uint32_t)M, ma, base_seed(ma) + (uint64_t)p, (uint32_t)h, mdl);
        if (ma.models && by == 0 && h < ma.modelH) store_model(ma, (size_t)p * ma.modelH + h, mdl);
        if (MODE == PS_REPROJECTION_ERROR || MODE == PS_EUCLIDEAN_AND_REPROJECTION_ERROR)
            inverse_rigid_general(mdl, inv);
    }
    int cnt = 0;
    if (MODE == PS_MAHALANOBIS_ERROR) valid = false;
    const float4 *__restrict__ pa = recA + rbase;
    const float4 *__restrict__ pb = recB + rbase;
    const float4 *__restrict__ pc = recC + rbase;
    if (MODE == PS_EUCLIDEAN_ERROR || MODE == PS_ADAPTIVE_ERROR) {
#pragma unroll 4
        for (int m = m0; m < m1; ++m) {
            float4 A = pa[m], B = pb[m];
            score_accumulate<MODE, false>(mdl, inv, k, A, B, A, cnt);
        }
    } else {
        const float cmax = cmaxArr[p].x;
        const float fmaxK = fmaxf(fmaxf(fabsf(k.fx), fabsf(k.fy)), 1.0f);
        const bool hoisted = wave_all(hi_bound_holds(mdl, cmax, fmaxK) && hi_bound_holds(inv, cmax, fmaxK));
        if (hoisted) {
            for (int m = m0; m < m1; ++m) {
                float4 A = pa[m], B = pb[m], C = pc[m];
                score_accumulate<MODE, true>(mdl, inv, k, A, B, C, cnt);
            }
        } else {
            for (int m = m0; m < m1; ++m) {
                float4 A = pa[m], B = pb[m], C = pc[m];
                score_accumulate<MODE, false>(mdl, inv, k, A, B, C, cnt);
            }
        }
    }
    if (h < H) {
        if (!valid) cnt = 0;
        if (msplit == 1)
            counts[(size_t)p * H + h] = cnt;
        else if (cnt)
            atomicAdd(&counts[(size_t)p * H + h], cnt);
    }
}

PS_D float wave_tree_sum(float v)
{
#if defined(__HIP_DEVICE_COMPILE__)
    v = v + __builtin_bit_cast(float, __builtin_amdgcn_update_dpp(0, __builtin_bit_cast(int, v), 0x101, 0xF, 0xF, false));
    v = v + __builtin_bit_cast(float, __builtin_amdgcn_update_dpp(0, __builtin_bit_cast(int, v), 0x102, 0xF, 0xF, false));
    v = v + __builtin_bit_cast(float, __builtin_amdgcn_update_dpp(0, __builtin_bit_cast(int, v), 0x104, 0xF, 0xF, false));
    v = v + __builtin_bit_cast(float, __builtin_amdgcn_update_dpp(0, __builtin_bit_cast(int, v), 0x108, 0xF, 0xF, false));
    const int b = __builtin_bit_cast(int, v);
    const float r0 = __builtin_bit_cast(float, __builtin_amdgcn_readlane(b, 0));
    const float r16 = __builtin_bit_cast(float, __builtin_amdgcn_readlane(b, 16));
    const float r32 = __builtin_bit_cast(float, __builtin_amdgcn_readlane(b, 32));
    const float r48 = __builtin_bit_cast(float, __builtin_amdgcn_readlane(b, 48));
    return (r0 + r16) + (r32 + r48);
#else
    return v;
#endif
}

template <typename GetA, typename GetB> PS_D bool wave_umeyama(int k, int split, GetA getA, GetB getB, Rigid &mdl)
{
    const int lane = threadIdx.x & 63;
    const float one_over_n = 1.0f / (float)k;
    const int k1 = k < split ? k : split;
    const int jB = lane + (((k1 > lane ? k1 - lane : 0) + 63) >> 6 << 6);
    float ss[3] = {0.0f, 0.0f, 0.0f}, ds[3] = {0.0f, 0.0f, 0.0f};
    auto add1 = [&](const float4 &u, const float4 &v) {
        ss[0] = ss[0] + u.x; ss[1] = ss[1] + u.y; ss[2] = ss[2] + u.z;
        ds[0] = ds[0] + u.w; ds[1] = ds[1] + v.x; ds[2] = ds[2] + v.y;
    };
    {
        float4 u, v, un, vn;
        if (lane < k1) getA(lane, u, v);
        for (int j = lane; j < k1; j += 64) {
            if (j + 64 < k1) getA(j + 64, un, vn);
            add1(u, v);
            u = un;
            v = vn;
        }
        for (int j = jB; j < k; j += 64) {
            getB(j, u, v);
            add1(u, v);
        }
    }
    float sm[3], dm[3];
#pragma unroll
    for (int c = 0; c < 3; ++c) {
        sm[c] = wave_tree_sum(ss[c]) * one_over_n;
        dm[c] = wave_tree_sum(ds[c]) * one_over_n;
    }
    float acc[3][3];
#pragma unroll
    for (int r = 0; r < 3; ++r)
#pragma unroll
        for (int c = 0; c < 3; ++c) acc[r][c] = 0.0f;
    auto add2 = [&](const float4 &u, const float4 &v) {
        const float s[3] = {u.x, u.y, u.z}, d[3] = {u.w, v.x, v.y};
#pragma unroll
        for (int r = 0; r < 3; ++r)
#pragma unroll
            for (int c = 0; c < 3; ++c) acc[r][c] = acc[r][c] + (d[r] - dm[r]) * (s[c] - sm[c]);
// ... 1048 lines not shown
```

putslam_amd/csrc/ps_score_fast.h:

```cpp
#pragma once

#include "ps_kernels.h"

namespace psdev {

struct FastConsts {
    float fmaxK;
    float cmaxK;
    float thrUp;
    float bIn0;
    float cIn;
    float thr2Up;
    float cHi;
    int enabled;
};

struct EuclidConsts {
    float tbLo;
    float tbHi;
    int enabled;
};

constexpr int kQueueCap = 256;
constexpr float kEpsU = 5.9604644775390625e-08f;

typedef float v2f_t __attribute__((ext_vector_type(2)));

struct FastModel {
    v2f_t r00, r01, r02, t0;
    v2f_t r10, r11, r12, t1;
    v2f_t r20, r21, r22, t2;
};

PS_D void make_fast(const Rigid &m, const Rigid &inv, float fx, float fy, FastModel &f)
{
    f.r00 = v2f_t{fx * m.R[0][0], fx * inv.R[0][0]};
    f.r01 = v2f_t{fx * m.R[0][1], fx * inv.R[0][1]};
    f.r02 = v2f_t{fx * m.R[0][2], fx * inv.R[0][2]};
    f.r10 = v2f_t{fy * m.R[1][0], fy * inv.R[1][0]};
    f.r11 = v2f_t{fy * m.R[1][1], fy * inv.R[1][1]};
    f.r12 = v2f_t{fy * m.R[1][2], fy * inv.R[1][2]};
    f.r20 = v2f_t{m.R[2][0], inv.R[2][0]};
    f.r21 = v2f_t{m.R[2][1], inv.R[2][1]};
    f.r22 = v2f_t{m.R[2][2], inv.R[2][2]};
    f.t0 = v2f_t{fx * m.t[0], fx * inv.t[0]};
    f.t1 = v2f_t{fy * m.t[1], fy * inv.t[1]};
    f.t2 = v2f_t{m.t[2], inv.t[2]};
}

PS_D void model_norms(const Rigid &m, float &rho, float &tau)
{
#pragma unroll
    for (int i = 0; i < 3; ++i) {
        const float rs = (fabsf(m.R[i][0]) + fabsf(m.R[i][1])) + fabsf(m.R[i][2]);
        rho = rs > rho ? rs : (rs == rs ? rho : rs);
        const float ta = fabsf(m.t[i]);
        tau = ta > tau ? ta : (ta == ta ? tau : ta);
    }
}

PS_D v2f_t pk_fma(v2f_t a, v2f_t b, v2f_t c) { return __builtin_elementwise_fma(a, b, c); }
PS_D v2f_t limit_lower(v2f_t K, v2f_t q, v2f_t G)
{
    v2f_t r;
    asm("v_pk_fma_f32 %0, %1, %2, %3 op_sel:[0,0,1] op_sel_hi:[0,1,1]" : "=v"(r) : "v"(K), "v"(q), "v"(G));
    return r;
}
PS_D v2f_t limit_upper(v2f_t K, v2f_t q, v2f_t G)
{
    v2f_t r;
    asm("v_pk_fma_f32 %0, %1, %2, %3 op_sel:[1,0,0] op_sel_hi:[1,1,0]" : "=v"(r) : "v"(K), "v"(q), "v"(G));
    return r;
}

PS_D v2f_t fast_sq2(const FastModel &f, v2f_t px, v2f_t py, v2f_t pz, v2f_t kx, v2f_t ky, v2f_t &Zout)
{
    const v2f_t X = pk_fma(f.r00, px, pk_fma(f.r01, py, pk_fma(f.r02, pz, f.t0)));
    const v2f_t Y = pk_fma(f.r10, px, pk_fma(f.r11, py, pk_fma(f.r12, pz, f.t1)));
    const v2f_t Z = pk_fma(f.r20, px, pk_fma(f.r21, py, pk_fma(f.r22, pz, f.t2)));
    const v2f_t Au = pk_fma(kx, Z, X);
    const v2f_t Bv = pk_fma(ky, Z, Y);
    Zout = Z;
    return pk_fma(Au, Au, Bv * Bv);
}


constexpr int kPrefixFixed = kBlock;
constexpr int kPrefixAdaptive = 64;
constexpr int kStages = 3;
constexpr int kReorderTopMax = 16;
constexpr int kReorderMargin = 16;

struct StageArgs {
    int stage;
    int hBase, hCount;
    int listStride;
    const int32_t *listIn;
    const int32_t *countIn;
    int32_t *listOut;
    int32_t *countOut;
    const int32_t *perm;
    const float2 *frontRec;
    int margin, c2div;
    unsigned long long *validMask;
    int genOnly;
    int single;
    int gran;
    int loopGroups;
    const int32_t *prefInfo;
};

PS_D void wave_replay_prefix(const int32_t *__restrict__ cnts, int n, const SelectArgs &a, int M, int &best, int &limit,
                             int &bestIdx)
{
    const int lane = threadIdx.x & 63;
    bestIdx = -1;
    if (a.estimator == PS_EST_FIXED) {
        int b = 0;
        for (int i = lane; i < n; i += 64) b = max(b, (cnts[i] << 16) | (0xFFFF - i));
#pragma unroll
        for (int o = 32; o > 0; o >>= 1) b = max(b, __shfl_xor(b, o, 64));
        best = b >> 16;
        if (best > 0) bestIdx = 0xFFFF - (b & 0xFFFF);
        limit = a.H;
        return;
    }
    int pos = 0;
    best = 0;
    limit = a.iter0;
    for (;;) {
        const int lim = limit < n ? limit : n;
        unsigned found = 0xFFFFFFFFu;
        for (int i = pos + lane; i < lim; i += 64)
            if (cnts[i] > best) {
                found = (unsigned)i;
                break;
            }
#pragma unroll
        for (int o = 32; o > 0; o >>= 1) {
            const unsigned other = (unsigned)__shfl_xor((int)found, o, 64);
            found = other < found ? other : found;
        }
        if (found == 0xFFFFFFFFu) break;
        best = cnts[found];
        bestIdx = (int)found;
        pos = (int)found + 1;
        limit = a.estimator == PS_EST_USAC ? usac_limit(a, (unsigned)best, (unsigned)M)
                                           : ransac_limit(a, (float)best / (float)M);
    }
}

PS_D void stage_range(const StageArgs &st, int M, int best0, int &lo, int &hi)
{
    const int stage = st.stage;
    const bool reordered = st.perm != nullptr;
    int c1 = M, c2 = M;
    if (best0 > 0 && !st.single) {
        const int miss = M - best0;
        if (reordered) {
            const int g1 = st.gran - 1;
            c1 = (miss + st.margin + g1) & ~g1;
            if (c1 >= M - M / 8) c1 = M;
            if (c1 < M) {
                const int c64 = (c1 + 63) & ~63;
                const int step = ((M - c64) / st.c2div + 63) & ~63;
                c2 = c64 + (step > 0 ? step : 64);
                if (c2 >= M - M / 16) c2 = M;
            }
        } else {
            c1 = (miss + miss / 7 + 32 + 63) & ~63;
            if (c1 >= M - M / 8) c1 = M;
            if (c1 < M) {
                c2 = (c1 + (M - c1) / 2 + 63) & ~63;
                if (c2 >= M - M / 16) c2 = M;
            }
        }
    }
    static_assert(kStages == 3, "three pruned stages");
    lo = stage == 1 ? 0 : (stage == 2 ? c1 : c2);
    hi = stage == 1 ? c1 : (stage == 2 ? c2 : M);
}

PS_D int hFirstOfWave(int h, int lane) { return __builtin_amdgcn_readfirstlane(h); }

PS_D void stage_prefix(const int32_t *__restrict__ cnts, int nPrefix, const SelectArgs &sa, int M, int *s_pref, int &best0,
                       int &hLimit, const int32_t *__restrict__ prefInfo = nullptr)
{
    if (prefInfo != nullptr) {
        best0 = prefInfo[0];
        hLimit = best0 > 0 ? prefInfo[1] : sa.H;
        return;
    }
    if ((threadIdx.x >> 6) == 0) {
        int b, l, bi;
        wave_replay_prefix(cnts, nPrefix, sa, M, b, l, bi);
        if ((threadIdx.x & 63) == 0) {
            s_pref[0] = b;
            s_pref[1] = l;
        }
    }
    __syncthreads();
    best0 = __builtin_amdgcn_readfirstlane(s_pref[0]);
    hLimit = best0 > 0 ? __builtin_amdgcn_readfirstlane(s_pref[1]) : sa.H;
}

PS_D void stage_append(bool alive, int h, int32_t *__restrict__ listOut, int32_t *__restrict__ countOut, int p, int stride)
{
    const unsigned long long am = __builtin_amdgcn_ballot_w64(alive);
    if (am == 0ull) return;
    const int lane = threadIdx.x & 63;
    int base = 0;
    if (lane == __builtin_ctzll(am)) base = atomicAdd(&countOut[p], __popcll(am));
    base = __builtin_amdgcn_readlane(base, __builtin_ctzll(am));
    if (alive) listOut[(size_t)p * stride + base + lanes_below(am)] = h;
}

PS_D int stage_hypothesis_again(bool list, const StageArgs &st, int base, int slot, int p, int H)
{
    asm volatile("" : "+s"(base));
    if (!list) return st.hBase + base + slot;
    const int i = base + slot;
    return i < st.countIn[p] ? st.listIn[(size_t)p * st.listStride + i] : 0x7FFFFFFF;
}

PS_D int list_cover(int n) { return n <= 64 ? 64 : (n <= 128 ? 128 : kBlock); }

template <int MODE, bool BIG, int KIND>
PS_D bool score_fast_pass(const float4 *__restrict__ recA, const float4 *__restrict__ recB, const float4 *__restrict__ recC,
                          const float4 *__restrict__ recE, const float2 *__restrict__ recF,
                          const float2 *__restrict__ pairBound, const ModelArgs &ma, const ScoreConsts &k,
                          const FastConsts &fc, const EuclidConsts &ec, const SelectArgs &sa, const StageArgs &st, int H, int cap,
                          int msplit, int32_t *__restrict__ counts, unsigned long long *__restrict__ dbg, const unsigned bx,
                          const unsigned by, const int p, const int M)
{
    constexpr bool EUCLID = MODE == PS_EUCLIDEAN_AND_REPROJECTION_ERROR;
    __shared__ float s_mdl[12][kBlock];
    __shared__ uint32_t s_q[kBlock / 64][kQueueCap];
    __shared__ int s_cnt[kBlock];
    __shared__ int s_tot[kBlock];
    __shared__ int s_pref[2];

    int tid = threadIdx.x;
    if (KIND == 2) asm volatile("" : "+v"(tid));
    const int lane = tid & 63;
    const int wv = __builtin_amdgcn_readfirstlane(tid >> 6);
    const size_t rbase = (size_t)p * cap;
    int32_t *__restrict__ cout = counts + (size_t)p * H;
    int h = st.hBase + (int)bx * kBlock + tid;
    int hEnd = st.hBase + st.hCount;
    const int npair = (M + 1) >> 1;
    int m0 = 2 * (int)(((long long)npair * by) / msplit);
    int m1 = 2 * (int)(((long long)npair * (by + 1)) / msplit);
    m1 = m1 < M ? m1 : M;
    int best0 = 0;
    constexpr bool LIST = KIND == 2;
    constexpr bool pruned = KIND >= 1;
    int cover = kBlock, slot = tid, part = 0;
    int mStageEnd = m1;
    if (LIST) {
        s_tot[tid] = 0;
        __syncthreads();
    }
    if (pruned) {
        int hLimit;
        stage_prefix(cout, st.hBase, sa, M, s_pref, best0, hLimit,
                     st.prefInfo != nullptr ? st.prefInfo + 4 * p : nullptr);
        stage_range(st, M, best0, m0, m1);
        {
            const int blockEnd = st.hBase + ((int)bx + 1) * kBlock;
            if (!LIST && ma.models != nullptr && (blockEnd < hEnd ? blockEnd : hEnd) > ma.modelH) m1 = M;
        }
        mStageEnd = m1;
        if (m0 >= m1) return true;
        if (!LIST) {
            hEnd = hEnd < hLimit ? hEnd : hLimit;
        } else {
            if (msplit > 1) {
                const int blen = (((m1 - m0 + msplit - 1) / msplit) + 63) & ~63;
                m0 += (int)by * blen;
                m1 = m1 < m0 + blen ? m1 : m0 + blen;
                if (m0 >= m1) return false;
            }
            const int n = st.countIn[p];
            cover = list_cover(n);
            part = __builtin_amdgcn_readfirstlane(tid / cover);
            slot = tid - part * cover;
            const int i = (int)bx * cover + slot;
            hEnd = 0x7FFFFFFF;
            h = i < n ? st.listIn[(size_t)p * st.listStride + i] : 0x7FFFFFFF;
            const int parts = kBlock / cover;
            const int plen = ((m1 - m0 + parts * 64 - 1) / (parts * 64)) * 64;
            m0 += part * plen;
            m1 = m1 < m0 + plen ? m1 : m0 + plen;
            m1 = m1 < m0 ? m0 : m1;
        }
        if (!LIST && st.hBase + (int)bx * kBlock >= hEnd) return true;
    }

    if (cover == kBlock && hFirstOfWave(h, lane) >= hEnd) return false;

    Rigid mdl;
    set_identity(mdl);
    bool valid = false;
    if (LIST) {
        if (h < hEnd) {
            load_model(ma, (size_t)p * ma.modelH + h, mdl);
            valid = true;
        }
    } else if (KIND == 0 && st.validMask != nullptr && !st.genOnly) {
        const unsigned long long vm = uniform64(st.validMask[(size_t)p * ((st.hCount + 63) >> 6) + (bx * (kBlock / 64) + wv)]);
        valid = h < hEnd && lane_in(vm);
        if (h < hEnd) load_model(ma, (size_t)p * ma.modelH + h, mdl);
    } else {
        if (h < hEnd) valid = gen_model(recA, recB, rbase, (uint32_t)M, ma, base_seed(ma) + (uint64_t)p, (uint32_t)h, mdl);
        if (ma.models && by == 0 && !pruned) {
            const int hs = stage_hypothesis_again(false, st, (int)bx * kBlock, tid, p, H);
            if (hs < hEnd && hs < ma.modelH) store_model(ma, (size_t)p * ma.modelH + hs, mdl);
        }
        if (KIND == 0 && st.genOnly) {
            const unsigned long long vm = __builtin_amdgcn_ballot_w64(valid);
            if (lane == 0) st.validMask[(size_t)p * ((st.hCount + 63) >> 6) + (bx * (kBlock / 64) + wv)] = vm;
            return false;
        }
    }
#pragma unroll
    for (int i = 0; i < 3; ++i) {
#pragma unroll
        for (int j = 0; j < 3; ++j) s_mdl[3 * i + j][tid] = mdl.R[i][j];
        s_mdl[9 + i][tid] = mdl.t[i];
    }
    s_cnt[tid] = 0;

    const float4 *__restrict__ pa = recA + rbase;
    const float4 *__restrict__ pb = recB + rbase;
    const float4 *__restrict__ pc = recC + rbase;
    const float4 *__restrict__ pe = recE + rbase;
    const float2 *__restrict__ pf = recF + rbase * 5;
    const int32_t *__restrict__ pperm = (pruned && st.perm != nullptr) ? st.perm + rbase : nullptr;
    auto orig = [&](int m) { return pperm != nullptr ? pperm[m] : m; };
    const float2 pbnd = pairBound[p];
    const float cmax = pbnd.x, umax = pbnd.y;

    int cnt = 0;
    {
        FastModel F;
        v2f_t KL, GG;
        float S;
        float U[3][4];
        float loE = 0.0f, hiE = 0.0f;
        const float lam = 1.05f * kEpsU * (14.0f * fc.fmaxK + 11.0f * umax + 4.0f * fc.cmaxK);
        const float g = 1.4143f * lam + 8.0f * kEpsU * fc.thrUp;
        auto rebuild = [&]() {
            Rigid md, iv;
#pragma unroll
            for (int i = 0; i < 3; ++i) {
#pragma unroll
                for (int j = 0; j < 3; ++j) md.R[i][j] = s_mdl[3 * i + j][tid];
                md.t[i] = s_mdl[9 + i][tid];
            }
            inverse_rigid_general(md, iv);
            make_fast(md, iv, k.fx, k.fy, F);
            float rho2 = 0.0f, tau2 = 0.0f;
            model_norms(md, rho2, tau2);
            model_norms(iv, rho2, tau2);
            S = (rho2 * cmax + tau2) * 1.001f;
            const float G = S * g;
            const float eps = 2.0f / cmax;
            const float TG = (fc.thrUp * G) * 1.00001f;
            const float cQ = (TG * eps) * 1.00001f;
            const float G2p = ((TG / eps) * 1.00001f + (G * G) * 1.0001f) * 1.00002f;
            KL = v2f_t{fc.bIn0 * 0.999999f - cQ, fc.thr2Up * 1.000001f + cQ};
            GG = v2f_t{G2p, -G2p};
            if (EUCLID) {
#pragma unroll
                for (int i = 0; i < 3; ++i) {
#pragma unroll
                    for (int j = 0; j < 3; ++j) U[i][j] = md.R[i][j];
                    U[i][3] = md.t[i];
                }
                float rhoE = 0.0f, tauE = 0.0f;
                model_norms(md, rhoE, tauE);
                const float aE = ((rhoE * cmax + tauE) * 1.001f) * (12.7f * kEpsU);
                const float xl = ec.tbLo - aE;
                loE = xl > 0.0f ? (xl * xl) * (1.0f - 8.0f * kEpsU) : -1.0f;
                const float yh = ec.tbHi + aE * (1.0f + 4.0f * kEpsU);
                hiE = (yh * yh) * (1.0f + 8.0f * kEpsU);
            }
        };
        rebuild();
        const bool boundsOk = fc.enabled != 0 && S * fc.fmaxK <= kDivHi && S >= 1.0e-20f && umax <= 1.0e7f &&
                              (!EUCLID || (ec.enabled != 0 && cmax <= 1.0e15f));
        if (!wave_all(boundsOk)) {
            Rigid md, iv;
#pragma unroll
            for (int i = 0; i < 3; ++i) {
#pragma unroll
                for (int j = 0; j < 3; ++j) md.R[i][j] = s_mdl[3 * i + j][tid];
                md.t[i] = s_mdl[9 + i][tid];
            }
            inverse_rigid_general(md, iv);
            for (int m = m0; m < m1; ++m) {
                const int mo = orig(m);
                const float4 A = pa[mo], B = pb[mo], C = pc[mo];
                score_accumulate<MODE, false>(md, iv, k, A, B, C, cnt);
            }
        } else {
        int qn = 0;
        unsigned long long parked = 0;

        auto drain = [&]() {
            __builtin_amdgcn_fence(__ATOMIC_ACQ_REL, "wavefront");
            for (int e = lane; e < qn; e += 64) {
                const uint32_t ent = s_q[wv][e];
                const int t = wv * 64 + (int)(ent & 63u), m = orig((int)(ent >> 6));
                Rigid md, iv;
#pragma unroll
                for (int i = 0; i < 3; ++i) {
#pragma unroll
                    for (int j = 0; j < 3; ++j) md.R[i][j] = s_mdl[3 * i + j][t];
                    md.t[i] = s_mdl[9 + i][t];
                }
                inverse_rigid_general(md, iv);
                const float4 A = pa[m], B = pb[m], C = pc[m];
                if (inlier_test<MODE>(md, iv, k, A, B, C)) atomicAdd(&s_cnt[t], 1);
            }
            __builtin_amdgcn_fence(__ATOMIC_ACQ_REL, "wavefront");
            parked += (unsigned long long)qn;
            qn = 0;
        };

        const unsigned long long execAll = __builtin_amdgcn_ballot_w64(true);
        struct Rec {
            unsigned long long q[5];
        };
        auto pair64 = [](float lo, float hi) {
            return (unsigned long long)__builtin_bit_cast(uint32_t, lo) | ((unsigned long long)__builtin_bit_cast(uint32_t, hi) << 32);
        };
        auto load_rec = [&](int m, const unsigned long long *__restrict__ rp) {
            Rec r;
            if (BIG) {
#pragma unroll
                for (int i = 0; i < 5; ++i) r.q[i] = rp[i];
            } else {
                const float4 A = pa[m], B = pb[m], E = pe[m];
                r.q[0] = pair64(B.x, A.x); r.q[1] = pair64(B.y, A.y); r.q[2] = pair64(B.z, A.z);
                r.q[3] = pair64(E.x, E.y); r.q[4] = pair64(E.z, E.w);
            }
            return r;
        };
        auto eval = [&](const Rec &r) -> unsigned long long {
            v2f_t Z;
            const v2f_t e0 = __builtin_bit_cast(v2f_t, r.q[0]), e1 = __builtin_bit_cast(v2f_t, r.q[1]),
                        e2 = __builtin_bit_cast(v2f_t, r.q[2]), e3 = __builtin_bit_cast(v2f_t, r.q[3]),
                        e4 = __builtin_bit_cast(v2f_t, r.q[4]);
            const v2f_t ss = fast_sq2(F, e0, e1, e2, e3, e4, Z);
            const float cxm = e0.x, cym = e1.x, czm = e2.x, pxm = e0.y, pym = e1.y, pzm = e2.y;
            const v2f_t q = Z * Z;
            const v2f_t lo = limit_lower(KL, q, GG);
            const v2f_t hi = limit_upper(KL, q, GG);
            const float se = ss.x, sn = ss.y, loe = lo.x, lon = lo.y, hie = hi.x, hin = hi.y;
            unsigned long long mIn =
                __builtin_amdgcn_ballot_w64(se < loe) & __builtin_amdgcn_ballot_w64(sn < lon);
            unsigned long long mOut =
                __builtin_amdgcn_ballot_w64(se > hie) | __builtin_amdgcn_ballot_w64(sn > hin);
            if (EUCLID) {
                const float d0 = __builtin_fmaf(U[0][0], cxm, __builtin_fmaf(U[0][1], cym, __builtin_fmaf(U[0][2], czm, U[0][3]))) - pxm;
                const float d1 = __builtin_fmaf(U[1][0], cxm, __builtin_fmaf(U[1][1], cym, __builtin_fmaf(U[1][2], czm, U[1][3]))) - pym;
                const float d2 = __builtin_fmaf(U[2][0], cxm, __builtin_fmaf(U[2][1], cym, __builtin_fmaf(U[2][2], czm, U[2][3]))) - pzm;
                const float sE = __builtin_fmaf(d0, d0, __builtin_fmaf(d1, d1, d2 * d2));
                mIn &= __builtin_amdgcn_ballot_w64(sE < loE);
                mOut |= __builtin_amdgcn_ballot_w64(sE > hiE);
            }
            add_mask(cnt, mIn);
            return mIn | mOut;
        };
        auto bx2 = [](float v) { return v2f_t{v, v}; };
        auto not_out2 = [&](const float2 *__restrict__ fr, unsigned long long &ua, unsigned long long &ub) {
            const unsigned long long *__restrict__ e = reinterpret_cast<const unsigned long long *>(fr);
            const unsigned long long q0 = e[0], q1 = e[1], q2 = e[2], q3 = e[3], q4 = e[4];
            const v2f_t cx = __builtin_bit_cast(v2f_t, q0), cy = __builtin_bit_cast(v2f_t, q1), cz = __builtin_bit_cast(v2f_t, q2),
                        kx = __builtin_bit_cast(v2f_t, q3), ky = __builtin_bit_cast(v2f_t, q4);
            const v2f_t X = pk_fma(bx2(F.r00.x), cx, pk_fma(bx2(F.r01.x), cy, pk_fma(bx2(F.r02.x), cz, bx2(F.t0.x))));
            const v2f_t Y = pk_fma(bx2(F.r10.x), cx, pk_fma(bx2(F.r11.x), cy, pk_fma(bx2(F.r12.x), cz, bx2(F.t1.x))));
            const v2f_t Z = pk_fma(bx2(F.r20.x), cx, pk_fma(bx2(F.r21.x), cy, pk_fma(bx2(F.r22.x), cz, bx2(F.t2.x))));
            const v2f_t A = pk_fma(kx, Z, X), B = pk_fma(ky, Z, Y);
            const v2f_t ss = pk_fma(A, A, B * B);
            const v2f_t q = Z * Z;
            const v2f_t hi = limit_upper(KL, q, GG);
            const float sa = ss.x, sb = ss.y, ha = hi.x, hb2 = hi.y;
            ua = __builtin_amdgcn_ballot_w64(sa > ha);
            ub = __builtin_amdgcn_ballot_w64(sb > hb2);
        };
        constexpr bool PRE = KIND == 1;
        int mFront = m0;
        const float2 *__restrict__ pfr = reinterpret_cast<const float2 *>(recE) + (size_t)p * ((size_t)((cap + 1) >> 1) * 5);
        if (PRE && st.frontRec != nullptr && st.prefInfo != nullptr) {
            const int f = __builtin_amdgcn_readfirstlane(st.prefInfo[4 * p + 2]);
            mFront = f < m1 ? f : m1;
        }
        const unsigned long long *__restrict__ rp = reinterpret_cast<const unsigned long long *>(pf) + 5 * (size_t)m0;
        const float2 *__restrict__ fr2 = pfr + 5 * (size_t)(m0 >> 1);
        const int mPairs = m0 + ((m1 - m0) & ~1);
        int frontParkTrips = 0;
        for (int m = m0; m < mPairs; m += 2, rp += 10, fr2 += (PRE ? 5 : 0)) {
            unsigned long long ua, ub;
            if (PRE && m + 2 <= mFront) {
                not_out2(fr2, ua, ub);
            } else {
                Rec ra = load_rec(m, rp), rb = load_rec(m + 1, rp + 5);
                asm volatile("" : "+s"(ra.q[0]), "+s"(ra.q[1]), "+s"(ra.q[2]), "+s"(ra.q[3]), "+s"(ra.q[4]), "+s"(rb.q[0]),
                             "+s"(rb.q[1]), "+s"(rb.q[2]), "+s"(rb.q[3]), "+s"(rb.q[4]));
                ua = eval(ra);
                ub = eval(rb);
            }
            if ((ua & ub) != execAll) {
                if (PRE && m + 2 <= mFront) ++frontParkTrips;
#pragma nounroll
                for (int j = 0; j < 2; ++j) {
                    const unsigned long long mU = execAll & ~(j ? ub : ua);
                    if (mU == 0ull) continue;
                    const int n = __popcll(mU);
                    if (qn + n > kQueueCap) {
                        drain();
                        rebuild();
                    }
                    if (lane_in(mU)) s_q[wv][qn + lanes_below(mU)] = ((uint32_t)(m + j) << 6) | (uint32_t)lane;
                    qn += n;
                }
            }
        }
        if (mPairs < m1) {
            const int n = __popcll(execAll);
            if (qn + n > kQueueCap) drain();
            s_q[wv][qn + lanes_below(execAll)] = ((uint32_t)mPairs << 6) | (uint32_t)lane;
            qn += n;
        }
        drain();
        cnt += s_cnt[tid];
        if (dbg != nullptr && lane == 0) {
            atomicAdd(&dbg[0], parked);
            atomicAdd(&dbg[1], (unsigned long long)(m1 - m0) * 64ull);
            if (PRE) {
                const int frontTrips = mFront > m0 ? ((mFront < mPairs ? mFront : mPairs) - m0) >> 1 : 0;
                atomicAdd(&dbg[3], (unsigned long long)frontParkTrips);
                atomicAdd(&dbg[2], (unsigned long long)(frontTrips - frontParkTrips));
            }
        }
        }
    }
    int tidE = tid;
    asm volatile("" : "+v"(tidE));
    if (LIST && cover < kBlock) {
        if (part > 0 && h < hEnd) atomicAdd(&s_tot[slot], cnt);
        __syncthreads();
        if (part == 0) cnt += s_tot[slot];
    }
    if (pruned) {
        h = stage_hypothesis_again(LIST, st, (int)bx * cover, slot, p, H);
        const bool mine = h < hEnd && part == 0;
        if (LIST && msplit > 1) {
            if (mine && valid && cnt) atomicAdd(&cout[h], cnt);
            return false;
        }
        const int cnt0 = (LIST && mine) ? cout[h] : 0;
        const int total = valid ? cnt0 + cnt : 0;
        if (mine) cout[h] = total;
        const bool alive = mine && valid && total + (M - mStageEnd) > best0;
        if (!LIST && ma.models && h < ma.modelH && (alive || (mine && mStageEnd >= M))) {
            Rigid md;
#pragma unroll
            for (int i = 0; i < 3; ++i) {
#pragma unroll
                for (int j = 0; j < 3; ++j) md.R[i][j] = s_mdl[3 * i + j][tidE];
                md.t[i] = s_mdl[9 + i][tidE];
            }
            store_model(ma, (size_t)p * ma.modelH + h, md);
        }
        if (st.stage < kStages && mStageEnd < M) stage_append(alive, h, st.listOut, st.countOut, p, st.listStride);
        return false;
    }
    h = stage_hypothesis_again(false, st, (int)bx * kBlock, tid, p, H);
    if (h < hEnd) {
        if (!valid) cnt = 0;
        if (msplit == 1)
            cout[h] = cnt;
        else if (cnt)
            atomicAdd(&cout[h], cnt);
    }
    return false;
}

template <int MODE, bool BIG, int KIND = 0, bool LOOP = false>
__global__ __launch_bounds__(kBlock, (KIND == 2 || LOOP) ? 5 : 8) void ps_ransac_score_fast(
    const float4 *__restrict__ recA, const float4 *__restrict__ recB, const float4 *__restrict__ recC,
    const float4 *__restrict__ recE, const float2 *__restrict__ recF, const int32_t *__restrict__ mvalid,
    const float2 *__restrict__ pairBound,
    ModelArgs ma, ScoreConsts k, FastConsts fc, EuclidConsts ec, SelectArgs sa, StageArgs st, int H, int cap, int minRun,
    int msplit, int32_t *__restrict__ counts, unsigned long long *__restrict__ dbg)
{
    static_assert(MODE == PS_REPROJECTION_ERROR || MODE == PS_EUCLIDEAN_AND_REPROJECTION_ERROR,
                  "the metrics with a reprojection test");
    static_assert(!LOOP || KIND == 1, "the looping form is stage 1's");
    const unsigned blocks = (unsigned)((st.hCount + kBlock - 1) / kBlock);
    const unsigned hb = LOOP ? (unsigned)st.loopGroups : blocks;
    const unsigned L = xcd_remap(blockIdx.x, gridDim.x);
    const unsigned bx = L % hb, by = (L / hb) % (unsigned)msplit;
    const int p = (int)(L / (hb * (unsigned)msplit));
    const int M = mvalid[p];
    if (M < minRun) return;
    if (LOOP) {
        for (unsigned b = bx; b < blocks; b += hb) {
            if (b != bx) __syncthreads();
            if (score_fast_pass<MODE, BIG, KIND>(recA, recB, recC, recE, recF, pairBound, ma, k, fc, ec, sa, st, H, cap, msplit,
                                                 counts, dbg, b, by, p, M))
                break;
        }
    } else if (KIND == 2) {
        const int n = st.countIn[p];
        const int cover = list_cover(n);
        for (unsigned b = bx; (int)b * cover < n; b += hb) {
            if (b != bx) __syncthreads();
            score_fast_pass<MODE, BIG, KIND>(recA, recB, recC, recE, recF, pairBound, ma, k, fc, ec, sa, st, H, cap, msplit, counts,
                                             dbg, b, by, p, M);
        }
    } else
        score_fast_pass<MODE, BIG, KIND>(recA, recB, recC, recE, recF, pairBound, ma, k, fc, ec, sa, st, H, cap, msplit, counts, dbg,
                                         bx, by, p, M);
}

template <int MODE>
__global__ __launch_bounds__(kBlock) void ps_stage_reorder(const float4 *__restrict__ recA, const float4 *__restrict__ recB,
                                                           const float4 *__restrict__ recC, const float2 *__restrict__ recF,
                                                           const int32_t *__restrict__ mvalid, ModelArgs ma, ScoreConsts k,
                                                           SelectArgs sa, int prefix, int nTopMax, int bailGran, int bailMargin,
                                                           int H, int cap, int minRun,
                                                           const int32_t *__restrict__ counts, float2 *__restrict__ recF2,
                                                           int32_t *__restrict__ perm, int32_t *__restrict__ prefInfo,
                                                           float2 *__restrict__ frontRec, unsigned *__restrict__ bailCount)
{
    constexpr bool EUCLID_REC = MODE == PS_EUCLIDEAN_ERROR || MODE == PS_ADAPTIVE_ERROR;
    constexpr int RF = MODE == PS_ADAPTIVE_ERROR ? 16 : 12;
    constexpr int kMaxChunks = PS_MAX_KPTS / kBlock;
    __shared__ int s_top[kReorderTopMax + 1];
    __shared__ uint8_t s_rej[PS_MAX_KPTS];
    __shared__ float s_vote[kReorderTopMax][24];
    __shared__ int s_tab[(kReorderTopMax + 2) * kMaxChunks * (kBlock / 64)];
    const int p = blockIdx.x;
    const int M = mvalid[p];
    if (M < minRun) return;
    const int tid = threadIdx.x, lane = tid & 63;
    const int wv = __builtin_amdgcn_readfirstlane(tid >> 6);
    const size_t rbase = (size_t)p * cap;
    const int32_t *__restrict__ cnts = counts + (size_t)p * H;
    if (wv == 0) {
        int b, l, bi;
        wave_replay_prefix(cnts, prefix, sa, M, b, l, bi);
        if (lane == 0) {
            prefInfo[4 * p] = b;
            prefInfo[4 * p + 1] = l;
            prefInfo[4 * p + 2] = 0;
            prefInfo[4 * p + 3] = 0;
        }
        int n = 0;
        const bool idle = b > 0 && l <= prefix;
        bool bail = false;
        if (bailGran > 0 && b > 0) {
            const int c1 = (M - b + bailMargin + bailGran - 1) & ~(bailGran - 1);
            bail = c1 >= M - M / 8;
        }
        if (b > 0 && !idle && !bail) {
            int key[4];
#pragma unroll
            for (int j = 0; j < 4; ++j) {
                const int i = lane + 64 * j;
                key[j] = (i < prefix && cnts[i] > 0) ? ((cnts[i] << 16) | (0xFFFF - i)) : 0;
            }
            for (; n < nTopMax; ++n) {
                int m = max(max(key[0], key[1]), max(key[2], key[3]));
#pragma unroll
                for (int o = 32; o > 0; o >>= 1) m = max(m, __shfl_xor(m, o, 64));
                if (m == 0) break;
                if (lane == 0) s_top[1 + n] = 0xFFFF - (m & 0xFFFF);
#pragma unroll
                for (int j = 0; j < 4; ++j)
                    if (key[j] == m) key[j] = 0;
            }
        }
        if (lane == 0) {
            s_top[0] = idle ? -1 : n;
            if (bail) prefInfo[4 * p + 3] = 1;
            if (bailCount != nullptr) {
                atomicAdd(&bailCount[0], 1u);
                if (bail || b <= 0) atomicAdd(&bailCount[1], 1u);
            }
        }
    }
    __syncthreads();
    const int nTop = s_top[0];
    if (nTop < 0) return;
    const float4 *__restrict__ pa = recA + rbase;
    const float4 *__restrict__ pb = recB + rbase;
    const float4 *__restrict__ pc = recC + rbase;
    if (tid < nTop) {
        Rigid mdl, inv;
        load_model(ma, (size_t)p * ma.modelH + s_top[1 + tid], mdl);
        inverse_rigid_general(mdl, inv);
#pragma unroll
        for (int i = 0; i < 3; ++i) {
#pragma unroll
            for (int j = 0; j < 3; ++j) {
                s_vote[tid][3 * i + j] = mdl.R[i][j];
                s_vote[tid][12 + 3 * i + j] = inv.R[i][j];
            }
            s_vote[tid][9 + i] = mdl.t[i];
            s_vote[tid][21 + i] = inv.t[i];
        }
    }
    __syncthreads();
    for (int m = tid; m < M; m += kBlock) {
        const float4 A = pa[m], B = pb[m], C = pc[m];
        int rej = 0;
        bool far = (MODE == PS_REPROJECTION_ERROR || MODE == PS_EUCLIDEAN_AND_REPROJECTION_ERROR) && nTop >= 1;
        for (int t = 0; t < nTop; ++t) {
            Rigid mdl, inv;
#pragma unroll
            for (int i = 0; i < 3; ++i) {
#pragma unroll
                for (int j = 0; j < 3; ++j) {
                    mdl.R[i][j] = s_vote[t][3 * i + j];
                    inv.R[i][j] = s_vote[t][12 + 3 * i + j];
                }
                mdl.t[i] = s_vote[t][9 + i];
                inv.t[i] = s_vote[t][21 + i];
            }
            rej += inlier_test<MODE>(mdl, inv, k, A, B, C) ? 0 : 1;
            if (MODE == PS_REPROJECTION_ERROR || MODE == PS_EUCLIDEAN_AND_REPROJECTION_ERROR) {
                float ex, ey, ez, pu, pv;
                xform(mdl, B.x, B.y, B.z, ex, ey, ez);
                project(ex, ey, ez, k.fx, k.fy, k.cx, k.cy, pu, pv);
                const float du = pu - C.x, dv = pv - C.y;
                far = far && (du * du + dv * dv > 16.0f * (float)k.boundR);
            }
        }
        s_rej[m] = (uint8_t)(far && rej == nTop ? 0 : 1 + nTop - rej);
    }
    const int nB = nTop + 2;
    const int nChunks = (M + kBlock - 1) / kBlock;
    for (int c = 0; c < nChunks; ++c) {
        const int m = c * kBlock + tid;
        const int d = m < M ? (int)s_rej[m] : -1;
        for (int b = 0; b < nB; ++b) {
            const unsigned long long bal = __builtin_amdgcn_ballot_w64(d == b);
            if (lane == 0) s_tab[(b * nChunks + c) * (kBlock / 64) + wv] = __popcll(bal);
        }
    }
    __syncthreads();
    if (wv == 0) {
        const int n = nB * nChunks * (kBlock / 64);
        int carry = 0;
        for (int e0 = 0; e0 < n; e0 += 64) {
            const int e = e0 + lane;
            const int v = e < n ? s_tab[e] : 0;
            int inc = v;
#pragma unroll
            for (int o = 1; o < 64; o <<= 1) {
                const int u = __shfl_up(inc, o, 64);
                if (lane >= o) inc += u;
            }
            if (e < n) s_tab[e] = carry + inc - v;
            carry += __shfl(inc, 63, 64);
        }
    }
    __syncthreads();
    const int front = s_tab[(1 * nChunks) * (kBlock / 64)];
    if (tid == 0) prefInfo[4 * p + 2] = front;
    float *__restrict__ frOut =
        (EUCLID_REC || frontRec == nullptr) ? nullptr : reinterpret_cast<float *>(frontRec) + (size_t)p * ((size_t)((cap + 1) >> 1) * 10);
    const float *__restrict__ gIn = reinterpret_cast<const float *>(recF) + (size_t)p * ((size_t)((cap + 1) >> 1) * RF);
    float *__restrict__ gOut = reinterpret_cast<float *>(recF2) + (size_t)p * ((size_t)((cap + 1) >> 1) * RF);
    for (int c = 0; c < nChunks; ++c) {
        const int m = c * kBlock + tid;
        const int d = m < M ? (int)s_rej[m] : -1;
        int pos = 0;
        for (int b = 0; b < nB; ++b) {
            const unsigned long long bal = __builtin_amdgcn_ballot_w64(d == b);
            if (d == b) pos = s_tab[(b * nChunks + c) * (kBlock / 64) + wv] + lanes_below(bal);
        }
        if (m < M) {
            perm[rbase + pos] = m;
            if (EUCLID_REC) {
                const float *src = gIn + (size_t)(m >> 1) * RF + (m & 1);
                float *dst = gOut + (size_t)(pos >> 1) * RF + (pos & 1);
#pragma unroll
                for (int i = 0; i < RF; i += 2) dst[i] = src[i];
            } else {
                const float2 *src = recF + 5 * (rbase + m);
                float2 *dst = recF2 + 5 * (rbase + pos);
#pragma unroll
                for (int i = 0; i < 5; ++i) dst[i] = src[i];
                if (frOut != nullptr && pos < front) {
                    float *fd = frOut + (size_t)(pos >> 1) * 10 + (pos & 1);
#pragma unroll
                    for (int i = 0; i < 5; ++i) fd[2 * i] = src[i].x;
                }
            }
        }
    }
    if (EUCLID_REC && (M & 1)) {
        __syncthreads();
        if (tid == 0) {
            float *g = gOut + (size_t)(M >> 1) * RF;
            for (int i = 0; i < RF; i += 2) g[i + 1] = g[i];
        }
    }
}

}
```

Measured before the change: 580,400 frame-pairs/s.

## Regroup doomed stage-1 hypotheses into their own wavefronts for one-direction pretest

The reorder kernel now writes a per-match doom flag, and stage 1 of the fixed-estimator reprojection scorer uses it to sort hypotheses inside each block so that doomed ones share wavefronts. Those wavefronts run the cheap one-direction pretest over the whole stage range rather than only the front. To support this, the reorder kernel extends frontRec out to the stage-1 end, and models are rebuilt from stored sample indices. The aim is to stop divergent wavefronts mixing doomed and live lanes, which forces full evaluation. The cost is extra shared-memory shuffles and block syncs per block, plus extra global writes for the flags and the longer frontRec.

```diff
diff --git a/profiles/r07a/frontshare.py b/profiles/r07a/frontshare.py
--- /dev/null
+++ b/profiles/r07a/frontshare.py
@@ -0,0 +1,30 @@
+import os, sys
+ROOT = os.path.dirname(os.path.dirname(os.path.dirname(os.path.abspath(__file__))))
+sys.path.insert(0, ROOT)
+import numpy as np
+from putslam_amd import api, synth
+from putslam_amd._abi import EST_FIXED, TUM_FR1_K, default_ransac_params, make_config
+from putslam_amd.device_batch import FrameSetDevice, PairBatchDevice, run_pairs
+seq = synth.make_sequence(500, 2000, config=3, index=0)
+prm = default_ransac_params(1)
+cfg, _ = make_config(EST_FIXED, 4096, seed=0xB0B0)
+c = api.Context(0)
+c.set_option("score_stats", 1)
+fs = FrameSetDevice(seq["desc"], seq["pts"], seq["nkpts"])
+pb = PairBatchDevice(seq["pairs"], fs.max_kpts)
+run_pairs(c, prm, cfg, TUM_FR1_K, fs, pb)
+g = pb.download()
+P = len(seq["pairs"])
+perm, front = c.stage_order(P, fs.max_kpts)
+surv = c.stage_survivors(P)
+st = c.score_stats_ex()
+M = g["stats"]["numMatchesValid"].astype(np.float64)
+best = g["stats"]["bestInlierCount"].astype(np.float64)
+f = front / M
+print("pairs", P, "M mean %.1f  best count mean %.1f  miss mean %.1f  front mean %.1f (min %d max %d)  front/M mean %.4f  front/miss mean %.3f" %
+      (M.mean(), best.mean(), (M - best).mean(), front.mean(), front.min(), front.max(), f.mean(), (front / np.maximum(M - best, 1)).mean()))
+pd = 1 - (1 - f) ** 3
+print("expected doomed hypotheses share mean %.4f  -> doomed lanes per block of 256 mean %.1f ; pairs with >= 64: %d, >= 128: %d ; upper bound of doomed wavefront share (perfect packing) %.4f ; per-block floor(nD/64)/4 estimate %.4f" %
+      (pd.mean(), (256 * pd).mean(), int((256 * pd >= 64).sum()), int((256 * pd >= 128).sum()), pd.mean(), (np.floor(256 * pd / 64) / 4).mean()))
+print("survivors stage1 mean %.1f stage2 mean %.1f" % (surv[0].mean(), surv[1].mean()))
+print("counters", st)
diff --git a/profiles/r07a/gate.py b/profiles/r07a/gate.py
--- /dev/null
+++ b/profiles/r07a/gate.py
@@ -0,0 +1,50 @@
+import os, sys
+ROOT = os.path.dirname(os.path.dirname(os.path.dirname(os.path.abspath(__file__))))
+sys.path.insert(0, ROOT)
+import numpy as np
+from putslam_amd import api, synth
+from putslam_amd._abi import EST_FIXED, TUM_FR1_K, default_ransac_params, make_config
+from putslam_amd.device_batch import FrameSetDevice, PairBatchDevice, run_pairs
+
+
+def run(seq, prm, cfg, **opts):
+    c = api.Context(0)
+    for k, v in opts.items():
+        c.set_option(k.replace("__", "."), v)
+    c.set_option("score_stats", 1)
+    fs = FrameSetDevice(seq["desc"], seq["pts"], seq["nkpts"])
+    pb = PairBatchDevice(seq["pairs"], fs.max_kpts)
+    run_pairs(c, prm, cfg, TUM_FR1_K, fs, pb)
+    g = pb.download()
+    st = c.score_stats_ex()
+    c.close()
+    return g, st
+
+
+def same(a, b):
+    return (a["pose"].tobytes() == b["pose"].tobytes() and a["inlierMask"].tobytes() == b["inlierMask"].tobytes()
+            and a["stats"].tobytes() == b["stats"].tobytes())
+
+
+for ev in (1, 2):
+    for H in (512, 600, 768):
+        seq = synth.make_sequence(4, 384, config=3, index=7 + H, inlier_frac=0.7, noise=0.004)
+        prm = default_ransac_params(ev)
+        cfg, _ = make_config(EST_FIXED, H, seed=99)
+        g0, s0 = run(seq, prm, cfg, prune=2, debug__regroup=0)
+        g1, s1 = run(seq, prm, cfg, prune=2, debug__regroup=1)
+        gf, _ = run(seq, prm, cfg, prune=0)
+        print("small ev", ev, "H", H, "same01", same(g0, g1), "sameFull", same(g1, gf), "stats0", s0, "stats1", s1, flush=True)
+
+seq = synth.make_sequence(500, 2000, config=3, index=0)
+prm = default_ransac_params(1)
+cfg, _ = make_config(EST_FIXED, 4096, seed=0xB0B0)
+g0, s0 = run(seq, prm, cfg, debug__regroup=0)
+g1, s1 = run(seq, prm, cfg, debug__regroup=1)
+print("bench same01", same(g0, g1))
+print("bench stats regroup=0", s0)
+print("bench stats regroup=1", s1)
+w, d, t0, t1 = s1[4], s1[5], s1[6], s1[7]
+print("stage-1 wavefronts %d doomed %d share %.3f ; beyond-front trips %d parking %d share %.4f" %
+      (w, d, d / max(w, 1), t0 + t1, t1, t1 / max(t0 + t1, 1)))
+print("front trips: regroup0 %d/%d  regroup1 %d/%d ; parked evals %d vs %d of %d" % (s0[3], s0[2] + s0[3], s1[3], s1[2] + s1[3], s0[0], s1[0], s1[1]))
diff --git a/profiles/r07a/summarise_rocprof.py b/profiles/r07a/summarise_rocprof.py
--- /dev/null
+++ b/profiles/r07a/summarise_rocprof.py
@@ -0,0 +1,30 @@
+import csv, glob, sys, collections, statistics as st
+kind, d = sys.argv[1], sys.argv[2]
+import re
+def short(n):
+    m = re.search(r"(ps_\w+)(<[^>]*>)?", n)
+    return (m.group(1) + (m.group(2) or "")) if m else n[:40]
+if kind == "trace":
+    f = [x for x in glob.glob(d + "/**/*kernel_trace.csv", recursive=True)][0]
+    dur = collections.defaultdict(list)
+    for r in csv.DictReader(open(f)):
+        dur[short(r["Kernel_Name"])].append((int(r["End_Timestamp"]) - int(r["Start_Timestamp"])) / 1e3)
+    for k, v in sorted(dur.items(), key=lambda kv: -sum(kv[1])):
+        v2 = v[len(v) // 2:]
+        q = sorted(v2)
+        print("%-32s n %5d  median %9.2f us  p10 %9.2f  p90 %9.2f  min %9.2f max %9.2f  total %10.1f us" %
+              (k, len(v), st.median(v2), q[len(q) // 10], q[(9 * len(q)) // 10], q[0], q[-1], sum(v)))
+else:
+    f = [x for x in glob.glob(d + "/**/*counter_collection.csv", recursive=True)][0]
+    val = collections.defaultdict(lambda: collections.defaultdict(float))
+    grid = {}
+    for r in csv.DictReader(open(f)):
+        key = (short(r["Kernel_Name"]), r["Dispatch_Id"])
+        val[key][r["Counter_Name"]] += float(r["Counter_Value"])
+        grid[key] = r.get("Grid_Size")
+    per = collections.defaultdict(lambda: collections.defaultdict(list))
+    for (k, _), cs in val.items():
+        for c, v in cs.items():
+            per[k][c].append(v)
+    for k in sorted(per):
+        print(k, "dispatches", len(next(iter(per[k].values()))), "  ".join("%s median %.4g" % (c, st.median(v)) for c, v in sorted(per[k].items())))
diff --git a/putslam_amd/csrc/ps_capi.hip b/putslam_amd/csrc/ps_capi.hip
--- a/putslam_amd/csrc/ps_capi.hip
+++ b/putslam_amd/csrc/ps_capi.hip
@@ -407,6 +407,8 @@
             PS_ENSURE(ctx->permBuf, n * sizeof(int32_t));
             PS_ENSURE(ctx->prefInfo, (size_t)4 * P * sizeof(int32_t));
             PS_ENSURE(ctx->frontRec, (size_t)P * ((cap + 1) / 2) * 10 * sizeof(float));
+            if (ctx->pretest != 0 && ctx->regroup != 0 && pl.sa.estimator == PS_EST_FIXED && pl.score == Scoring::Reproj)
+                PS_ENSURE(ctx->doomFlag, n);
         }
         pl.pa.zeroSurvA = (int32_t *)ctx->survN.p;
         pl.pa.zeroSurvB = (int32_t *)ctx->survN.p + P;
@@ -492,6 +494,7 @@
     auto list_rsplit = [&](int stage) { return (pl.reorder && stage == kStages) ? kListRsplit3 : 1; };
     const bool usePretest = pl.reorder && ctx->pretest != 0 &&
                             (pl.mode == PS_EUCLIDEAN_AND_REPROJECTION_ERROR || pl.mode == PS_REPROJECTION_ERROR);
+    const bool useRegroup = usePretest && ctx->regroup != 0 && pl.sa.estimator == PS_EST_FIXED && ctx->doomFlag.p != nullptr;
     const int blocks1 = (pl.H - pl.prefix + kBlock - 1) / kBlock;
     int loopGroups = 0;
     if (pl.sa.estimator != PS_EST_FIXED && blocks1 > 64) {
@@ -512,6 +515,7 @@
         if (stage >= 1 && pl.reorder) st.perm = (const int32_t *)ctx->permBuf.p;
         if (stage >= 1 && pl.reorder) st.prefInfo = (const int32_t *)ctx->prefInfo.p;
         if (stage == 1 && usePretest) st.frontRec = (const float2 *)ctx->frontRec.p;
+        if (stage == 1 && useRegroup) st.doomFlag = (const uint8_t *)ctx->doomFlag.p;
         st.listStride = pl.ma.modelH;
         st.loopGroups = stage == 1 ? loopGroups : 0;
         st.single = pl.lastStage == 1 ? 1 : 0;
@@ -534,9 +538,11 @@
         hipLaunchKernelGGL(ps_stage_reorder<MODE>, dim3((unsigned)P), dim3(kBlock), 0, ctx->stream, (const float4 *)ctx->recA.p,
                            (const float4 *)ctx->recB.p, (const float4 *)ctx->recC.p, (const float2 *)ctx->recF.p,
                            (const int32_t *)ctx->mvalid.p, pl.ma, pl.sc, pl.sa, pl.prefix, ctx->reorderTop,
-                           (ctx->bail != 0 && pl.score == Scoring::Euclid) ? 64 : 0, ctx->reorderMargin, pl.H, c.cap, pl.minRun,
+                           (ctx->bail != 0 && pl.score == Scoring::Euclid) ? 64 : 0, ctx->reorderMargin,
+                           useRegroup ? kReorderGran : 0, pl.lastStage == 1 ? 1 : 0, pl.H, c.cap, pl.minRun,
                            (const int32_t *)ctx->counts.p, (float2 *)ctx->recF2.p, (int32_t *)ctx->permBuf.p,
                            (int32_t *)ctx->prefInfo.p, usePretest ? (float2 *)ctx->frontRec.p : (float2 *)nullptr,
+                           useRegroup ? (uint8_t *)ctx->doomFlag.p : (uint8_t *)nullptr,
                            pl.bailWatch ? (unsigned *)ctx->bailCnt.p + 2 * pl.bailSlot : (unsigned *)nullptr);
     if (loopGroups > 0)
         k3(Kind<1, true>{}, stage_args(1), (unsigned)loopGroups, 1);
diff --git a/putslam_amd/csrc/ps_context.cpp b/putslam_amd/csrc/ps_context.cpp
--- a/putslam_amd/csrc/ps_context.cpp
+++ b/putslam_amd/csrc/ps_context.cpp
@@ -123,6 +123,7 @@
     {"gensplit", "GENSPLIT", &PsContext::genSplit, 0, 1, "gensplit: 0 (stage 0 as one launch) or 1 (models, then the sweep)", true},
     {"singlerest", "SINGLEREST", &PsContext::singleRest, 0, 1, "singlerest: 0 (three stages) or 1 (one stage after the prefix, adaptive schedules)", true},
     {"pretest", "PRETEST", &PsContext::pretest, 0, 1, "pretest: 0 or 1 (stage 1's one-direction pre-test)", true},
+    {"regroup", "REGROUP", &PsContext::regroup, 0, 1, "regroup: 0 or 1 (stage 1 groups doomed hypotheses into wavefronts of their own)", true},
     {"list_g2", "LISTG2", &PsContext::listGroups2, 0, 64, "list_g2: 0 (automatic) .. 64 work-groups per pair of stage 2", true},
     {"prefix", "PREFIX", &PsContext::forcePrefix, 0, 256, "prefix: 0 (default) or 64, 128, 192, 256 hypotheses of stage 0 (fixed schedule)", true},
     {"reorder_top", "REORDER_TOP", &PsContext::reorderTop, 1, kPsReorderTopMax, "reorder_top: 1 .. 16 voters", true},
@@ -224,7 +225,7 @@
     if (!ctx) return;
     (void)hipSetDevice(ctx->device);
     (void)hipStreamSynchronize(ctx->stream);
-    Buf *all[] = {&ctx->keys, &ctx->recA, &ctx->recB, &ctx->recC, &ctx->recD, &ctx->recE, &ctx->recF, &ctx->recShadow, &ctx->models, &ctx->survA, &ctx->survB, &ctx->survN, &ctx->recF2, &ctx->permBuf, &ctx->prefInfo, &ctx->frontRec, &ctx->validMask, &ctx->stamps, &ctx->dbgCnt, &ctx->bailCnt, &ctx->counts, &ctx->mvalid,
+    Buf *all[] = {&ctx->keys, &ctx->recA, &ctx->recB, &ctx->recC, &ctx->recD, &ctx->recE, &ctx->recF, &ctx->recShadow, &ctx->models, &ctx->survA, &ctx->survB, &ctx->survN, &ctx->recF2, &ctx->permBuf, &ctx->prefInfo, &ctx->doomFlag, &ctx->frontRec, &ctx->validMask, &ctx->stamps, &ctx->dbgCnt, &ctx->bailCnt, &ctx->counts, &ctx->mvalid,
                   &ctx->cmax, &ctx->idxList, &ctx->raw, &ctx->xq, &ctx->tabR, &ctx->tabU, &ctx->sDesc, &ctx->sNk,
                   &ctx->sMatches, &ctx->sNumM, &ctx->sMask, &ctx->sPose, &ctx->sStats,
                   &ctx->sMisc0, &ctx->sMisc1, &ctx->sMisc2, &ctx->exFlag, &ctx->exPar, &ctx->viewChunks, &ctx->levelTab, &ctx->poseSets, &ctx->loopPairs, &ctx->l2Keys, &ctx->l2Img, &ctx->l2Norms, &ctx->l2List, &ctx->l2ListLo, &ctx->l2Count, &ctx->l2Stat};
@@ -288,7 +289,7 @@
     if (strcmp(name, "hopeless") == 0) return ctx->hopeless;
     if (strcmp(name, "arena_mib") == 0) {
         const Buf *all[] = {&ctx->keys, &ctx->recA, &ctx->recB, &ctx->recC, &ctx->recD, &ctx->recE, &ctx->recF, &ctx->models,
-                            &ctx->survA, &ctx->survB, &ctx->survN, &ctx->recF2, &ctx->permBuf, &ctx->prefInfo, &ctx->frontRec,
+                            &ctx->survA, &ctx->survB, &ctx->survN, &ctx->recF2, &ctx->permBuf, &ctx->prefInfo, &ctx->doomFlag, &ctx->frontRec,
                             &ctx->validMask, &ctx->stamps, &ctx->dbgCnt, &ctx->bailCnt, &ctx->counts, &ctx->mvalid, &ctx->cmax,
                             &ctx->idxList, &ctx->raw, &ctx->xq, &ctx->tabR, &ctx->tabU, &ctx->sDesc, &ctx->sNk, &ctx->sMatches,
                             &ctx->sNumM, &ctx->sMask, &ctx->sPose, &ctx->sStats, &ctx->sMisc0, &ctx->sMisc1, &ctx->sMisc2, &ctx->exFlag, &ctx->exPar, &ctx->viewChunks, &ctx->levelTab, &ctx->poseSets, &ctx->loopPairs, &ctx->l2Keys, &ctx->l2Img, &ctx->l2Norms, &ctx->l2List, &ctx->l2ListLo, &ctx->l2Count, &ctx->l2Stat};
diff --git a/putslam_amd/csrc/ps_internal.h b/putslam_amd/csrc/ps_internal.h
--- a/putslam_amd/csrc/ps_internal.h
+++ b/putslam_amd/csrc/ps_internal.h
@@ -34,6 +34,7 @@
     Buf validMask;
     Buf frontRec;
     Buf prefInfo;
+    Buf doomFlag;
     Buf recF2, permBuf;
     Buf dbgCnt;
     Buf xq;
@@ -71,6 +72,7 @@
     int genSplit = 1;
     int singleRest = 1;
     int pretest = 1;
+    int regroup = 1;
     int listGroups2 = 0;
     int forcePrefix = 0;
     int bail = 1;
diff --git a/putslam_amd/csrc/ps_kernels.h b/putslam_amd/csrc/ps_kernels.h
--- a/putslam_amd/csrc/ps_kernels.h
+++ b/putslam_amd/csrc/ps_kernels.h
@@ -477,11 +477,9 @@
 }
 PS_D uint64_t base_seed(const ModelArgs &ma) { return ma.seedDev ? *ma.seedDev : ma.seed; }
 
-PS_D bool gen_model(const float4 *__restrict__ recA, const float4 *__restrict__ recB, size_t rbase, uint32_t M,
-                    const ModelArgs &ma, uint64_t pairSeed, uint32_t h, Rigid &mdl)
-{
-    uint32_t idx[3];
-    sample_triplet(pairSeed, ma.raw, h, M, idx);
+PS_D bool model_from_sample(const float4 *__restrict__ recA, const float4 *__restrict__ recB, size_t rbase,
+                            const uint32_t (&idx)[3], Rigid &mdl)
+{
     float src[3][3], dst[3][3];
 #pragma unroll
     for (int j = 0; j < 3; ++j) {
@@ -491,6 +489,13 @@
         src[j][0] = B.x; src[j][1] = B.y; src[j][2] = B.z;
     }
     return umeyama3(src, dst, mdl);
+}
+PS_D bool gen_model(const float4 *__restrict__ recA, const float4 *__restrict__ recB, size_t rbase, uint32_t M,
+                    const ModelArgs &ma, uint64_t pairSeed, uint32_t h, Rigid &mdl)
+{
+    uint32_t idx[3];
+    sample_triplet(pairSeed, ma.raw, h, M, idx);
+    return model_from_sample(recA, recB, rbase, idx, mdl);
 }
 
 struct ScoreConsts {
diff --git a/putslam_amd/csrc/ps_score_fast.h b/putslam_amd/csrc/ps_score_fast.h
--- a/putslam_amd/csrc/ps_score_fast.h
+++ b/putslam_amd/csrc/ps_score_fast.h
@@ -108,6 +108,7 @@
     int gran;
     int loopGroups;
     const int32_t *prefInfo;
+    const uint8_t *doomFlag;
 };
 
 PS_D void wave_replay_prefix(const int32_t *__restrict__ cnts, int n, const SelectArgs &a, int M, int &best, int &limit,
@@ -150,17 +151,29 @@
     }
 }
 
+PS_D int reordered_stage1_end(int M, int best0, int gran, int margin)
+{
+    const int g1 = gran - 1;
+    const int c1 = (M - best0 + margin + g1) & ~g1;
+    return c1 >= M - M / 8 ? M : c1;
+}
+PS_D int stage1_end(bool reordered, int single, int M, int best0, int gran, int margin)
+{
+    if (best0 <= 0 || single) return M;
+    if (reordered) return reordered_stage1_end(M, best0, gran, margin);
+    const int miss = M - best0;
+    const int c1 = (miss + miss / 7 + 32 + 63) & ~63;
+    return c1 >= M - M / 8 ? M : c1;
+}
+
 PS_D void stage_range(const StageArgs &st, int M, int best0, int &lo, int &hi)
 {
     const int stage = st.stage;
     const bool reordered = st.perm != nullptr;
-    int c1 = M, c2 = M;
+    const int c1 = stage1_end(reordered, st.single, M, best0, st.gran, st.margin);
+    int c2 = M;
     if (best0 > 0 && !st.single) {
-        const int miss = M - best0;
         if (reordered) {
-            const int g1 = st.gran - 1;
-            c1 = (miss + st.margin + g1) & ~g1;
-            if (c1 >= M - M / 8) c1 = M;
             if (c1 < M) {
                 const int c64 = (c1 + 63) & ~63;
                 const int step = ((M - c64) / st.c2div + 63) & ~63;
@@ -168,8 +181,6 @@
                 if (c2 >= M - M / 16) c2 = M;
             }
         } else {
-            c1 = (miss + miss / 7 + 32 + 63) & ~63;
-            if (c1 >= M - M / 8) c1 = M;
             if (c1 < M) {
                 c2 = (c1 + (M - c1) / 2 + 63) & ~63;
                 if (c2 >= M - M / 16) c2 = M;
@@ -257,6 +268,7 @@
     constexpr bool pruned = KIND >= 1;
     int cover = kBlock, slot = tid, part = 0;
     int mStageEnd = m1;
+    bool regroup = false;
     if (LIST) {
         s_tot[tid] = 0;
         __syncthreads();
@@ -268,7 +280,12 @@
         stage_range(st, M, best0, m0, m1);
         {
             const int blockEnd = st.hBase + ((int)bx + 1) * kBlock;
-            if (!LIST && ma.models != nullptr && (blockEnd < hEnd ? blockEnd : hEnd) > ma.modelH) m1 = M;
+            const bool whole = !LIST && ma.models != nullptr && (blockEnd < hEnd ? blockEnd : hEnd) > ma.modelH;
+            if (whole) m1 = M;
+            if (KIND == 1)
+                regroup = st.doomFlag != nullptr && st.frontRec != nullptr && st.prefInfo != nullptr && !whole &&
+                          st.loopGroups == 0 && sa.estimator == PS_EST_FIXED &&
+                          __builtin_amdgcn_readfirstlane(st.prefInfo[4 * p + 2]) > 0;
         }
         mStageEnd = m1;
         if (m0 >= m1) return true;
@@ -297,6 +314,52 @@
         if (!LIST && st.hBase + (int)bx * kBlock >= hEnd) return true;
     }
 
+    uint32_t sidx[3] = {0u, 0u, 0u};
+    bool doomedWave = false;
+    if (KIND == 1) {
+        if (h < hEnd) sample_triplet(base_seed(ma) + (uint64_t)p, ma.raw, (uint32_t)h, (uint32_t)M, sidx);
+        if (regroup) {
+            const bool live = h < hEnd;
+            bool doomed = false;
+            if (live) {
+                const uint8_t *__restrict__ fl = st.doomFlag + rbase;
+#pragma unroll
+                for (int j = 0; j < 3; ++j) doomed = doomed || (sidx[j] < (uint32_t)M && fl[sidx[j]] != 0);
+            }
+            const unsigned long long mD = __builtin_amdgcn_ballot_w64(doomed);
+            const unsigned long long mL = __builtin_amdgcn_ballot_w64(live && !doomed);
+            if (lane == 0) {
+                s_cnt[wv] = __popcll(mD);
+                s_cnt[4 + wv] = __popcll(mL);
+            }
+            __syncthreads();
+            int nD = 0, nL = 0, dBelow = 0, lBelow = 0;
+#pragma unroll
+            for (int w = 0; w < kBlock / 64; ++w) {
+                const int d = s_cnt[w], l = s_cnt[4 + w];
+                if (w < wv) { dBelow += d; lBelow += l; }
+                nD += d;
+                nL += l;
+            }
+            const int dl = lanes_below(mD), ll = lanes_below(mL);
+            const int pos = doomed ? dBelow + dl
+                                   : (live ? nD + lBelow + ll : nD + nL + (tid - dBelow - lBelow - dl - ll));
+            uint32_t *__restrict__ sx = &s_q[0][0];
+            sx[4 * pos] = live ? (uint32_t)h : 0x7FFFFFFFu;
+            sx[4 * pos + 1] = sidx[0];
+            sx[4 * pos + 2] = sidx[1];
+            sx[4 * pos + 3] = sidx[2];
+            __syncthreads();
+            h = (int)sx[4 * tid];
+            sidx[0] = sx[4 * tid + 1];
+            sidx[1] = sx[4 * tid + 2];
+            sidx[2] = sx[4 * tid + 3];
+            s_tot[tid] = h;
+            doomedWave = wave_all(tid < nD || h >= hEnd);
+            __builtin_amdgcn_fence(__ATOMIC_ACQ_REL, "wavefront");
+        }
+    }
+
     if (cover == kBlock && hFirstOfWave(h, lane) >= hEnd) return false;
 
     Rigid mdl;
@@ -312,7 +375,10 @@
         valid = h < hEnd && lane_in(vm);
         if (h < hEnd) load_model(ma, (size_t)p * ma.modelH + h, mdl);
     } else {
-        if (h < hEnd) valid = gen_model(recA, recB, rbase, (uint32_t)M, ma, base_seed(ma) + (uint64_t)p, (uint32_t)h, mdl);
+        if (KIND == 1) {
+            if (h < hEnd) valid = model_from_sample(recA, recB, rbase, sidx, mdl);
+        } else if (h < hEnd)
+            valid = gen_model(recA, recB, rbase, (uint32_t)M, ma, base_seed(ma) + (uint64_t)p, (uint32_t)h, mdl);
         if (ma.models && by == 0 && !pruned) {
             const int hs = stage_hypothesis_again(false, st, (int)bx * kBlock, tid, p, H);
             if (hs < hEnd && hs < ma.modelH) store_model(ma, (size_t)p * ma.modelH + hs, mdl);
@@ -498,10 +564,13 @@
             const int f = __builtin_amdgcn_readfirstlane(st.prefInfo[4 * p + 2]);
             mFront = f < m1 ? f : m1;
         }
+        const int mFrontOld = mFront;
+        if (PRE && doomedWave) mFront = m1;
         const unsigned long long *__restrict__ rp = reinterpret_cast<const unsigned long long *>(pf) + 5 * (size_t)m0;
         const float2 *__restrict__ fr2 = pfr + 5 * (size_t)(m0 >> 1);
         const int mPairs = m0 + ((m1 - m0) & ~1);
         int frontParkTrips = 0;
+        int doomParkTrips = 0;
         for (int m = m0; m < mPairs; m += 2, rp += 10, fr2 += (PRE ? 5 : 0)) {
             unsigned long long ua, ub;
             if (PRE && m + 2 <= mFront) {
@@ -514,7 +583,8 @@
                 ub = eval(rb);
             }
             if ((ua & ub) != execAll) {
-                if (PRE && m + 2 <= mFront) ++frontParkTrips;
+                if (PRE && m + 2 <= mFrontOld) ++frontParkTrips;
+                else if (PRE && m + 2 <= mFront) ++doomParkTrips;
 #pragma nounroll
                 for (int j = 0; j < 2; ++j) {
                     const unsigned long long mU = execAll & ~(j ? ub : ua);
@@ -541,9 +611,16 @@
             atomicAdd(&dbg[0], parked);
             atomicAdd(&dbg[1], (unsigned long long)(m1 - m0) * 64ull);
             if (PRE) {
-                const int frontTrips = mFront > m0 ? ((mFront < mPairs ? mFront : mPairs) - m0) >> 1 : 0;
+                const int frontTrips = mFrontOld > m0 ? ((mFrontOld < mPairs ? mFrontOld : mPairs) - m0) >> 1 : 0;
                 atomicAdd(&dbg[3], (unsigned long long)frontParkTrips);
                 atomicAdd(&dbg[2], (unsigned long long)(frontTrips - frontParkTrips));
+                atomicAdd(&dbg[4], 1ull);
+                if (doomedWave) {
+                    const int allTrips = mFront > m0 ? ((mFront < mPairs ? mFront : mPairs) - m0) >> 1 : 0;
+                    atomicAdd(&dbg[5], 1ull);
+                    atomicAdd(&dbg[7], (unsigned long long)doomParkTrips);
+                    atomicAdd(&dbg[6], (unsigned long long)(allTrips - frontTrips - doomParkTrips));
+                }
             }
         }
         }
@@ -557,6 +634,7 @@
     }
     if (pruned) {
         h = stage_hypothesis_again(LIST, st, (int)bx * cover, slot, p, H);
+        if (KIND == 1 && regroup) h = s_tot[tidE];
         const bool mine = h < hEnd && part == 0;
         if (LIST && msplit > 1) {
             if (mine && valid && cnt) atomicAdd(&cout[h], cnt);
@@ -632,16 +710,18 @@
 __global__ __launch_bounds__(kBlock) void ps_stage_reorder(const float4 *__restrict__ recA, const float4 *__restrict__ recB,
                                                            const float4 *__restrict__ recC, const float2 *__restrict__ recF,
                                                            const int32_t *__restrict__ mvalid, ModelArgs ma, ScoreConsts k,
-                                                           SelectArgs sa, int prefix, int nTopMax, int bailGran, int bailMargin,
-                                                           int H, int cap, int minRun,
+                                                           SelectArgs sa, int prefix, int nTopMax, int bailGran, int margin,
+                                                           int preGran, int single, int H, int cap, int minRun,
                                                            const int32_t *__restrict__ counts, float2 *__restrict__ recF2,
                                                            int32_t *__restrict__ perm, int32_t *__restrict__ prefInfo,
-                                                           float2 *__restrict__ frontRec, unsigned *__restrict__ bailCount)
+                                                           float2 *__restrict__ frontRec, uint8_t *__restrict__ doomFlag,
+                                                           unsigned *__restrict__ bailCount)
 {
     constexpr bool EUCLID_REC = MODE == PS_EUCLIDEAN_ERROR || MODE == PS_ADAPTIVE_ERROR;
     constexpr int RF = MODE == PS_ADAPTIVE_ERROR ? 16 : 12;
     constexpr int kMaxChunks = PS_MAX_KPTS / kBlock;
     __shared__ int s_top[kReorderTopMax + 1];
+    __shared__ int s_best;
     __shared__ uint8_t s_rej[PS_MAX_KPTS];
     __shared__ float s_vote[kReorderTopMax][24];
     __shared__ int s_tab[(kReorderTopMax + 2) * kMaxChunks * (kBlock / 64)];
@@ -656,6 +736,7 @@
         int b, l, bi;
         wave_replay_prefix(cnts, prefix, sa, M, b, l, bi);
         if (lane == 0) {
+            s_best = b;
             prefInfo[4 * p] = b;
             prefInfo[4 * p + 1] = l;
             prefInfo[4 * p + 2] = 0;
@@ -665,8 +746,7 @@
         const bool idle = b > 0 && l <= prefix;
         bool bail = false;
         if (bailGran > 0 && b > 0) {
-            const int c1 = (M - b + bailMargin + bailGran - 1) & ~(bailGran - 1);
-            bail = c1 >= M - M / 8;
+            bail = reordered_stage1_end(M, b, bailGran, margin) >= M;
         }
         if (b > 0 && !idle && !bail) {
             int key[4];
@@ -743,6 +823,7 @@
             }
         }
         s_rej[m] = (uint8_t)(far && rej == nTop ? 0 : 1 + nTop - rej);
+        if (doomFlag != nullptr) doomFlag[rbase + m] = (uint8_t)(far && rej == nTop ? 1 : 0);
     }
     const int nB = nTop + 2;
     const int nChunks = (M + kBlock - 1) / kBlock;
@@ -774,6 +855,7 @@
     __syncthreads();
     const int front = s_tab[(1 * nChunks) * (kBlock / 64)];
     if (tid == 0) prefInfo[4 * p + 2] = front;
+    const int preEnd = (preGran > 0 && front > 0) ? stage1_end(true, single, M, s_best, preGran, margin) : front;
     float *__restrict__ frOut =
         (EUCLID_REC || frontRec == nullptr) ? nullptr : reinterpret_cast<float *>(frontRec) + (size_t)p * ((size_t)((cap + 1) >> 1) * 10);
     const float *__restrict__ gIn = reinterpret_cast<const float *>(recF) + (size_t)p * ((size_t)((cap + 1) >> 1) * RF);
@@ -798,7 +880,7 @@
                 float2 *dst = recF2 + 5 * (rbase + pos);
 #pragma unroll
                 for (int i = 0; i < 5; ++i) dst[i] = src[i];
-                if (frOut != nullptr && pos < front) {
+                if (frOut != nullptr && pos < preEnd) {
                     float *fd = frOut + (size_t)(pos >> 1) * 10 + (pos & 1);
 #pragma unroll
                     for (int i = 0; i < 5; ++i) fd[2 * i] = src[i].x;
```

New measurement: 584,500 frame-pairs/s, median of 6. About the same (+0.7%).
